# UCL-CCS/SCEMa

Measured on AMD Instinct MI355X. Metric: stress_evals_per_sec, higher is better.
Workload: dtype f64; 1 GPU; 576 x PE-10368 OPLS replicas per update(), 10+100 MD steps each (dt 2 fs, 300 K, lj/cut/coul/long 12/9 + PPPM 1e-4 + SHAKE + NVT), persistent per-QP state, replica equilibrated for 2000 steps before the timed region; force_field=opls, strain_set=balanced (load/unload: odd updates take the draw with the opposite sign), n_sims=576, atoms_per_replica=10368, sims_on_rank0=576, allgathers=0

## Files before the change

### include/scema_md.h

```cpp
#ifndef SCEMA_MD_H
#define SCEMA_MD_H

#include <stdint.h>

#ifdef __cplusplus
extern "C" {
#endif

#define SCEMA_MD_OK 0
#define SCEMA_MD_ERR_ARG 1
#define SCEMA_MD_ERR_NOSTATE 2
#define SCEMA_MD_ERR_DEVICE 3
#define SCEMA_MD_ERR_BOX 4
#define SCEMA_MD_ERR_IO 5
#define SCEMA_MD_ERR_OVERFLOW 6

#define SCEMA_MD_NPART 8
#define SCEMA_MD_QP_NONE ((int32_t)0xFFFFFFFF)

typedef struct scema_md_engine scema_md_engine;

typedef struct {
  double cut_lj;
  double cut_coul;
// ... 90 lines not shown
int scema_md_comm_init_rccl(scema_md_engine *e, const void *id, int32_t rank, int32_t world);
typedef int (*scema_md_host_allgather_fn)(void *ctx, const void *send, void *recv, int64_t bytes_per_rank);
typedef int (*scema_md_host_send_fn)(void *ctx, const void *buf, int64_t bytes, int32_t dst_rank);
typedef int (*scema_md_host_recv_fn)(void *ctx, void *buf, int64_t bytes, int32_t src_rank);
int scema_md_comm_init_host(scema_md_engine *e, int32_t rank, int32_t world, scema_md_host_allgather_fn allgather,
                            scema_md_host_send_fn send, scema_md_host_recv_fn recv, void *ctx);
void scema_md_comm_destroy(scema_md_engine *e);
int32_t scema_md_comm_world(const scema_md_engine *e);
int32_t scema_md_comm_rank(const scema_md_engine *e);
int scema_md_comm_stats(const scema_md_engine *e, int64_t *allgathers, int64_t *migrations);
int64_t scema_md_comm_handshakes(const scema_md_engine *e);
int32_t scema_md_state_owner(const scema_md_engine *e, int32_t qp_id, const char *matid, int32_t replica);

int scema_md_last_plan(const scema_md_engine *e, int32_t n_sims, int32_t *owner, int32_t *pos, int32_t *cap);
#define SCEMA_MD_RESULT_TRAILER 2
void *scema_md_local_stress_device_ptr(scema_md_engine *e);
int32_t scema_md_local_stress_count(const scema_md_engine *e);
int32_t scema_md_local_result_doubles(const scema_md_engine *e);
int scema_md_copy_local_stress(scema_md_engine *e, void *dst, int32_t dst_on_device);
int scema_md_scatter_gathered(scema_md_engine *e, const double *gathered, scema_mdsim *sims, int32_t n_sims);
int scema_md_settle_update(scema_md_engine *e, int32_t failed);
int64_t scema_md_unsettled_updates(const scema_md_engine *e);

typedef struct scema_plan_dir scema_plan_dir;
scema_plan_dir *scema_plan_dir_create(void);
void scema_plan_dir_destroy(scema_plan_dir *d);
int scema_plan_update(scema_plan_dir *d, const scema_mdsim *sims, int32_t n_sims, const double *cost, int32_t world,
                      int32_t *owner, int32_t *pos, int32_t *cap, int32_t *moves ,
                      int32_t *n_moves, int32_t commit);

int scema_md_has_state(const scema_md_engine *e, int32_t qp_id, const char *matid, int32_t replica);
int scema_md_get_state(scema_md_engine *e, int32_t qp_id, const char *matid, int32_t replica,
                       double box[9], double *x, double *v);
int scema_md_set_state(scema_md_engine *e, int32_t qp_id, const char *matid, int32_t replica,
                       const double box[9], const double *x, const double *v);
int scema_md_drop_state(scema_md_engine *e, int32_t qp_id, const char *matid, int32_t replica);
int scema_md_save_state_file(scema_md_engine *e, int32_t qp_id, const char *matid, int32_t replica, const char *path);
int scema_md_load_state_file(scema_md_engine *e, int32_t qp_id, const char *matid, int32_t replica, const char *path);
int scema_md_save_state_lammps(scema_md_engine *e, int32_t qp_id, const char *matid, int32_t replica, const char *path,
                               double timestep, int64_t ntimestep);

int scema_md_save_state_dump(scema_md_engine *e, int32_t qp_id, const char *matid, int32_t replica, const char *path,
                             int64_t ntimestep, int32_t precise);

typedef struct {
  double timestep_length;
  double temperature;
  int32_t nsteps_sample;
  double strain_ampl;
  double strain_rate;
} scema_md_eqparams;
int scema_md_init_material(scema_md_engine *e, const char *matid, int32_t replica, const scema_md_eqparams *p,
                           double length[3], double stress[6], double stiff[36]);

typedef struct {
  int32_t nsteps_equil;
  double timestep_length;
  double temperature;
  int64_t seed;
} scema_md_equilparams;
int scema_md_equilibrate(scema_md_engine *e, const char *matid, int32_t replica, const scema_md_equilparams *p, double length[3],
                         double *info);

int scema_md_debug_minimize(scema_md_engine *e, int32_t qp_id, const char *matid, int32_t replica, double etol, double ftol,
                            int32_t maxiter, int32_t maxeval, double *info);
int scema_md_debug_run_nh(scema_md_engine *e, int32_t qp_id, const char *matid, int32_t replica, int32_t nsteps, double dt,
                          double t_start, double t_stop, int32_t npt, double p_target, double p_period, double *lavg);
int scema_md_debug_compute(scema_md_engine *e, int32_t qp_id, const char *matid, int32_t replica, int32_t use_shake,
                           double *f, double *energies, double *virials, double *info );
int scema_md_debug_skin_bands(scema_md_engine *e, int32_t pos, uint64_t *out, int32_t cap);
int scema_md_debug_rows(scema_md_engine *e, int32_t pos, int32_t *cnt, int32_t *rows, int64_t rows_cap, int32_t *info);
int scema_md_debug_run(scema_md_engine *e, int32_t qp_id, const char *matid, int32_t replica, int32_t nsteps,
                       double dt, double temperature, int32_t nvt, int32_t use_shake, const double *rates,
                       double *press_avg);

int scema_md_reax_configure(scema_md_engine *e, const char *ffield_path, const char *const *elements, int32_t n_elements,
                            double qeq_tol, double skin);
int scema_md_reax_activate(scema_md_engine *e, int32_t on);
int scema_md_reax_set(scema_md_engine *e, int32_t exact_gradient, int32_t terms, int32_t qeq_maxiter);
int scema_md_reax_concurrency(scema_md_engine *e, int32_t halves, int32_t overlap);
int scema_md_batch_split(scema_md_engine *e, int32_t on);
int scema_md_get_concurrency(const scema_md_engine *e, int32_t *out);
int scema_md_pppm_tiling(scema_md_engine *e, int32_t mode, int32_t lds_bytes);
int scema_md_pppm_paths(const scema_md_engine *e, int32_t out[8]);
int scema_md_pppm_tile_shape(const int32_t grid[3], int32_t lds_bytes, int32_t which , int32_t out[4]);
int scema_md_pppm_plan_count(const scema_md_engine *e);
int scema_md_reax_debug_compute(scema_md_engine *e, int32_t qp_id, const char *matid, int32_t replica, double *f, double *eparts,
                                double *virial, double *q, double *info);
int scema_md_reax_stats(const scema_md_engine *e, double *out);

int scema_md_sw_configure(scema_md_engine *e, const char *matid, const char *sw_path, const char *const *elements, int32_t n_elements,
                          int32_t energy_unit, double skin);
int scema_md_sw_debug_compute(scema_md_engine *e, int32_t qp_id, const char *matid, int32_t replica, double *f, double *e2, double *e3,
                              double *virial, double *info);
int scema_md_sw_read_params(const char *sw_path, const char *const *elements, int32_t n_elements, int32_t energy_unit, int32_t *n_kept,
                            int32_t *type_map, double *values, char *errbuf, int32_t errcap);

int scema_md_tersoff_configure(scema_md_engine *e, const char *matid, const char *path, const char *const *elements, int32_t n_elements,
                               int32_t energy_unit, double skin);
int scema_md_tersoff_debug_compute(scema_md_engine *e, int32_t qp_id, const char *matid, int32_t replica, double *f, double *e_rep,
                                   double *e_att, double *virial, double *info);
int scema_md_tersoff_read_params(const char *path, const char *const *elements, int32_t n_elements, int32_t energy_unit, int32_t *n_kept,
                                 int32_t *type_map, double *values, char *errbuf, int32_t errcap);

int scema_md_tersoff_mod_configure(scema_md_engine *e, const char *matid, const char *path, const char *const *elements, int32_t n_elements,
                                   int32_t energy_unit, double skin);
int scema_md_tersoff_mod_debug_compute(scema_md_engine *e, int32_t qp_id, const char *matid, int32_t replica, double *f, double *e_rep,
                                       double *e_att, double *virial, double *info);
int scema_md_tersoff_zbl_configure(scema_md_engine *e, const char *matid, const char *path, const char *const *elements, int32_t n_elements,
                                   int32_t energy_unit, double skin);
int scema_md_tersoff_zbl_debug_compute(scema_md_engine *e, int32_t qp_id, const char *matid, int32_t replica, double *f, double *e_rep,
                                       double *e_att, double *virial, double *info);
int scema_md_tersoff_mod_read_params(const char *path, const char *const *elements, int32_t n_elements, int32_t energy_unit, int32_t *n_kept,
                                     int32_t *type_map, double *values, char *errbuf, int32_t errcap);
int scema_md_tersoff_zbl_read_params(const char *path, const char *const *elements, int32_t n_elements, int32_t energy_unit, int32_t *n_kept,
                                     int32_t *type_map, double *values, char *errbuf, int32_t errcap);

int scema_md_eam_configure(scema_md_engine *e, const char *matid, const char *path, const char *const *elements, int32_t n_elements,
                           int32_t energy_unit, double skin);
int scema_md_eam_debug_compute(scema_md_engine *e, int32_t qp_id, const char *matid, int32_t replica, double *f, double *e_pair,
                               double *e_embed, double *virial, double *info);
int scema_md_eam_read_setfl(const char *path, const char *const *elements, int32_t n_elements, int32_t energy_unit, int32_t *n_kept,
                            int32_t *type_map, double *head, double *masses, double *tables, int64_t tables_cap, char *errbuf, int32_t errcap);

int scema_md_vashishta_configure(scema_md_engine *e, const char *matid, const char *path, const char *const *elements, int32_t n_elements,
                                 int32_t energy_unit, double skin);
int scema_md_vashishta_debug_compute(scema_md_engine *e, int32_t qp_id, const char *matid, int32_t replica, double *f, double *e2, double *e3,
                                     double *virial, double *info);
int scema_md_vashishta_read_params(const char *path, const char *const *elements, int32_t n_elements, int32_t energy_unit, int32_t *n_kept,
                                   int32_t *type_map, double *values, char *errbuf, int32_t errcap);

int scema_md_adp_configure(scema_md_engine *e, const char *matid, const char *path, const char *const *elements, int32_t n_elements,
                           int32_t energy_unit, double skin);
int scema_md_adp_debug_compute(scema_md_engine *e, int32_t qp_id, const char *matid, int32_t replica, double *f, double *e_pair, double *e_manybody,
                               double *virial, double *info);
int scema_md_adp_read_setfl(const char *path, const char *const *elements, int32_t n_elements, int32_t energy_unit, int32_t *n_kept,
                            int32_t *type_map, double *head, double *masses, double *tables, int64_t tables_cap, char *errbuf, int32_t errcap);

int scema_md_edip_configure(scema_md_engine *e, const char *matid, const char *path, const char *const *elements, int32_t n_elements,
                            int32_t energy_unit, double skin);
int scema_md_edip_debug_compute(scema_md_engine *e, int32_t qp_id, const char *matid, int32_t replica, double *f, double *e2, double *e3,
                                double *virial, double *info);
int scema_md_edip_read_params(const char *path, const char *const *elements, int32_t n_elements, int32_t energy_unit, int32_t *n_kept,
                              int32_t *type_map, double *values, char *errbuf, int32_t errcap);

typedef struct {
  int64_t pair_launches;
  double pair_ms;
  double pair_alg_bytes;
  int64_t md_steps;
  int64_t neigh_builds;
  double unique_pairs_per_sim;
  int64_t evals;
  double list_skin_mean;
  int64_t pair_sims;
  int64_t box_flips;
  int64_t rx_sweep_launches;
  double rx_sweep_ms;
  double rx_sweep_entries;
  double rx_sweep_rows;
  int64_t rx_sweep_col_bytes;
  double pair_union_ms;
  double rx_sweep_union_ms;
  int64_t rx_sweep_symmetric;
  int64_t row_cell_builds;
} scema_md_profile;
// ... 14 lines not shown
```

### scema_amd/capi.py

```python
from __future__ import annotations

import ctypes as C
import os

import numpy as np

_HERE = os.path.dirname(os.path.abspath(__file__))
LIB_PATH = os.path.join(_HERE, os.environ.get("SCEMA_MD_LIB") or ("libscema_md_asan.so" if os.environ.get("SCEMA_SANITIZE") == "1" else "libscema_md.so"))

NPART = 8
PARTS = ["lj", "coul", "bond", "angle", "dihedral", "improper", "kspace", "shake"]
QP_NONE = -1

SYMBOLS = [
    "scema_md_default_params", "scema_md_create", "scema_md_destroy", "scema_md_last_error",
    "scema_md_register_replica", "scema_md_load_replica_file", "scema_md_write_replica_file",
    "scema_md_load_lammps_data", "scema_md_convert_lammps_data",
    "scema_md_probe_lammps_restart", "scema_md_read_lammps_restart_atoms", "scema_md_load_lammps_restart",
    "scema_md_convert_lammps_restart", "scema_md_write_lammps_restart",
    "scema_md_strain_batch", "scema_md_strain", "scema_md_local_stress_device_ptr",
    "scema_md_local_stress_count", "scema_md_local_result_doubles", "scema_md_copy_local_stress", "scema_md_scatter_gathered", "scema_md_settle_update", "scema_md_has_state", "scema_md_get_state",
    "scema_md_set_state", "scema_md_drop_state", "scema_md_save_state_file", "scema_md_load_state_file", "scema_md_save_state_lammps",
    "scema_md_init_material", "scema_md_debug_compute", "scema_md_debug_run", "scema_md_debug_skin_bands", "scema_md_debug_rows", "scema_md_get_profile", "scema_md_env_overrides",
    "scema_md_comm_unique_id", "scema_md_comm_init_rccl", "scema_md_comm_init_host", "scema_md_comm_destroy",
    "scema_md_comm_world", "scema_md_comm_rank", "scema_md_comm_stats", "scema_md_comm_handshakes", "scema_md_state_owner", "scema_md_last_plan",
    "scema_plan_dir_create", "scema_plan_dir_destroy", "scema_plan_update", "scema_md_kspace_setup",
    "scema_md_save_state_dump", "scema_md_replica_natoms", "scema_md_save_replica_file", "scema_md_equilibrate", "scema_md_debug_minimize", "scema_md_debug_run_nh",
    "scema_md_reax_configure", "scema_md_reax_activate", "scema_md_reax_set", "scema_md_reax_concurrency", "scema_md_batch_split", "scema_md_get_concurrency", "scema_md_pppm_plan_count", "scema_md_pppm_tiling", "scema_md_pppm_paths", "scema_md_pppm_tile_shape", "scema_md_unsettled_updates", "scema_md_reax_debug_compute", "scema_md_reax_stats", "scema_md_box_fma_tflops",
    "scema_md_sw_configure", "scema_md_sw_debug_compute", "scema_md_sw_read_params",
    "scema_md_tersoff_configure", "scema_md_tersoff_debug_compute", "scema_md_tersoff_read_params",
    "scema_md_eam_configure", "scema_md_eam_debug_compute", "scema_md_eam_read_setfl",
    "scema_md_tersoff_mod_configure", "scema_md_tersoff_mod_debug_compute", "scema_md_tersoff_mod_read_params",
    "scema_md_tersoff_zbl_configure", "scema_md_tersoff_zbl_debug_compute", "scema_md_tersoff_zbl_read_params",
    "scema_md_vashishta_configure", "scema_md_vashishta_debug_compute", "scema_md_vashishta_read_params",
    "scema_md_adp_configure", "scema_md_adp_debug_compute", "scema_md_adp_read_setfl",
    "scema_md_edip_configure", "scema_md_edip_debug_compute", "scema_md_edip_read_params",
]
COMM_ID_BYTES = 128
HOST_ALLGATHER_FN = C.CFUNCTYPE(C.c_int, C.c_void_p, C.c_void_p, C.c_void_p, C.c_int64)
HOST_SEND_FN = C.CFUNCTYPE(C.c_int, C.c_void_p, C.c_void_p, C.c_int64, C.c_int32)
HOST_RECV_FN = C.CFUNCTYPE(C.c_int, C.c_void_p, C.c_void_p, C.c_int64, C.c_int32)


class EquilParams(C.Structure):
    _fields_ = [("nsteps_equil", C.c_int32), ("timestep_length", C.c_double), ("temperature", C.c_double), ("seed", C.c_int64)]


class Params(C.Structure):
    _fields_ = [("cut_lj", C.c_double), ("cut_coul", C.c_double), ("skin", C.c_double), ("neigh_delay", C.c_int32),
                ("kspace_accuracy", C.c_double), ("shake_tol", C.c_double), ("shake_maxiter", C.c_int32),
                ("shake_mass", C.c_double), ("t_period", C.c_double), ("t_chain", C.c_int32), ("device", C.c_int32),
                ("max_batch", C.c_int32), ("profile", C.c_int32), ("kspace_style", C.c_int32)]


_P = C.c_void_p


class System(C.Structure):
    _fields_ = [("natoms", C.c_int32), ("ntypes", C.c_int32), ("type", _P), ("charge", _P), ("mass", _P),
                ("eps", _P), ("sigma", _P),
                ("nbonds", C.c_int32), ("nbondtypes", C.c_int32), ("bond_atoms", _P), ("bond_type", _P), ("bond_coeff", _P),
                ("nangles", C.c_int32), ("nangletypes", C.c_int32), ("angle_atoms", _P), ("angle_type", _P), ("angle_coeff", _P),
                ("ndihedrals", C.c_int32), ("ndihedraltypes", C.c_int32), ("dihedral_atoms", _P), ("dihedral_type", _P),
                ("dihedral_coeff", _P),
                ("nimpropers", C.c_int32), ("nimpropertypes", C.c_int32), ("improper_atoms", _P), ("improper_type", _P),
                ("improper_coeff", _P),
                ("special_lj", C.c_double * 3), ("special_coul", C.c_double * 3), ("box", C.c_double * 9), ("x", _P), ("v", _P)]


class MDSim(C.Structure):
    _fields_ = [("qp_id", C.c_int32), ("most_recent_qp_id", C.c_int32), ("replica", C.c_int32), ("material", C.c_int32),
                ("matid", C.c_char_p), ("time_id", C.c_char_p), ("output_folder", C.c_char_p),
                ("restart_folder", C.c_char_p), ("scripts_folder", C.c_char_p), ("log_file", C.c_char_p),
                ("force_field", C.c_char_p),
                ("strain", C.c_double * 6), ("stiffness", C.c_double * 36),
                ("timestep_length", C.c_double), ("temperature", C.c_double), ("strain_rate", C.c_double),
                ("nsteps_sample", C.c_int32), ("output_homog", C.c_int32), ("checkpoint", C.c_int32),
                ("stress", C.c_double * 6), ("stress_updated", C.c_int32)]


class EqParams(C.Structure):
    _fields_ = [("timestep_length", C.c_double), ("temperature", C.c_double), ("nsteps_sample", C.c_int32),
                ("strain_ampl", C.c_double), ("strain_rate", C.c_double)]


class Profile(C.Structure):
    _fields_ = [("pair_launches", C.c_int64), ("pair_ms", C.c_double), ("pair_alg_bytes", C.c_double),
                ("md_steps", C.c_int64), ("neigh_builds", C.c_int64), ("unique_pairs_per_sim", C.c_double),
                ("evals", C.c_int64), ("list_skin_mean", C.c_double), ("pair_sims", C.c_int64), ("box_flips", C.c_int64),
                ("rx_sweep_launches", C.c_int64), ("rx_sweep_ms", C.c_double), ("rx_sweep_entries", C.c_double), ("rx_sweep_rows", C.c_double), ("rx_sweep_col_bytes", C.c_int64),
                ("pair_union_ms", C.c_double), ("rx_sweep_union_ms", C.c_double), ("rx_sweep_symmetric", C.c_int64),
                ("row_cell_builds", C.c_int64)]


_lib = None


def lib():
    global _lib
    if _lib is None:
        if not os.path.exists(LIB_PATH):
            raise RuntimeError(f"{LIB_PATH} is missing: run `python -c 'import __graft_entry__ as g; g.build()'` "
                               "(make -C scema_amd/csrc); the engine has no CPU fallback")
        L = C.CDLL(LIB_PATH)
        L.scema_md_last_error.restype = C.c_char_p
        L.scema_md_last_error.argtypes = [_P]
        L.scema_md_local_stress_device_ptr.restype = C.c_void_p
        L.scema_md_local_stress_device_ptr.argtypes = [_P]
        L.scema_md_local_stress_count.argtypes = [_P]
        L.scema_md_destroy.argtypes = [_P]
        L.scema_md_destroy.restype = None
# ... 254 lines not shown
    def save_state_file(self, qp, matid, replica, path):
        self._chk(lib().scema_md_save_state_file(self.h, C.c_int32(qp), matid.encode(), C.c_int32(replica), path.encode()))

    def save_state_lammps(self, qp, matid, replica, path, timestep=2.0, ntimestep=0):
        self._chk(lib().scema_md_save_state_lammps(self.h, C.c_int32(qp), matid.encode(), C.c_int32(replica), path.encode(),
                                                   C.c_double(timestep), C.c_int64(ntimestep)))

    def save_state_dump(self, qp, matid, replica, path, ntimestep=0, precise=True):
        self._chk(lib().scema_md_save_state_dump(self.h, C.c_int32(qp), matid.encode(), C.c_int32(replica), path.encode(), C.c_int64(ntimestep),
                                                 C.c_int32(1 if precise else 0)))

    def load_state_file(self, qp, matid, replica, path):
        self._chk(lib().scema_md_load_state_file(self.h, C.c_int32(qp), matid.encode(), C.c_int32(replica), path.encode()))

    def debug_compute(self, matid, replica, qp=QP_NONE, use_shake=False):
        n = self._natoms[(matid, replica)]
        f = np.zeros((n, 3)); e = np.zeros(NPART); w = np.zeros((NPART, 6)); info = np.zeros(8)
        self._chk(lib().scema_md_debug_compute(self.h, C.c_int32(qp), matid.encode(), C.c_int32(replica),
                                               C.c_int32(1 if use_shake else 0), _p(f), _p(e), _p(w), _p(info)))
        return f, e, w, dict(g_ewald=info[0], nk=int(info[1]), npairs=info[2], tdof=info[3], t_current=info[4],
                             maxneigh_seen=int(info[5]), maxneigh=int(info[6]), nclus=int(info[7]))

    def debug_run(self, matid, replica, nsteps, dt, temperature, qp=QP_NONE, nvt=True, use_shake=True, rates=None, sample=False):
        r = None if rates is None else np.ascontiguousarray(rates, np.float64)
        pavg = np.zeros(6) if sample else None
        self._chk(lib().scema_md_debug_run(self.h, C.c_int32(qp), matid.encode(), C.c_int32(replica), C.c_int32(nsteps),
                                           C.c_double(dt), C.c_double(temperature), C.c_int32(1 if nvt else 0),
                                           C.c_int32(1 if use_shake else 0), _p(r), _p(pavg)))
        return pavg

    def debug_skin_bands(self, pos=0):
        out = np.zeros(64, np.uint64)
        self._chk(lib().scema_md_debug_skin_bands(self.h, C.c_int32(pos), out.ctypes.data_as(C.c_void_p), C.c_int32(out.size)))
        k = int(out[0])
        return dict(K=k, listed=[int(v) for v in out[1:1 + k]], walked=[int(v) for v in out[1 + k:1 + 2 * k]],
                    rows=int(out[1 + 2 * k]), rows_open=int(out[2 + 2 * k]), rows_all_open=int(out[3 + 2 * k]))

    def debug_rows(self, pos=0, rows=True):
        info = np.zeros(6, np.int32)
        f = lib().scema_md_debug_rows
        f.argtypes = [_P, C.c_int32, C.c_void_p, C.c_void_p, C.c_int64, C.c_void_p]
        self._chk(f(self.h, pos, None, None, 0, info.ctypes.data))
        out = dict(n=int(info[0]), cap=int(info[1]), cells=int(info[2]), ncell=[int(v) for v in info[3:6]])
        if rows:
            cnt = np.zeros(out["n"], np.int32)
            tab = np.zeros((out["n"], out["cap"]), np.int32)
            self._chk(f(self.h, pos, cnt.ctypes.data, tab.ctypes.data, tab.size, info.ctypes.data))
            out.update(cnt=cnt, rows=tab)
        return out

    def init_material(self, matid, replica, dt=2.0, temperature=300.0, nss=100, strain_ampl=0.005, strain_rate=1e-4):
        p = EqParams(dt, temperature, nss, strain_ampl, strain_rate)
        length, stress, stiff = np.zeros(3), np.zeros(6), np.zeros(36)
        self._chk(lib().scema_md_init_material(self.h, matid.encode(), C.c_int32(replica), C.byref(p), _p(length), _p(stress), _p(stiff)))
        return length, stress, stiff.reshape(6, 6)

    def reax_configure(self, ffield: str, elements=("H", "C", "N", "O"), qeq_tol: float = 1e-6, skin: float = -1.0):
        arr = (C.c_char_p * len(elements))(*[e.encode() for e in elements])
        self._chk(lib().scema_md_reax_configure(self.h, ffield.encode(), arr, C.c_int32(len(elements)), C.c_double(qeq_tol), C.c_double(skin)))

    def reax_activate(self, on: bool = True):
        self._chk(lib().scema_md_reax_activate(self.h, C.c_int32(1 if on else 0)))

    def reax_set(self, exact_gradient: int = -1, terms: int = -1, qeq_maxiter: int = -1):
        self._chk(lib().scema_md_reax_set(self.h, C.c_int32(exact_gradient), C.c_int32(terms), C.c_int32(qeq_maxiter)))

    def reax_concurrency(self, halves: int = -1, overlap: int = -1):
        self._chk(lib().scema_md_reax_concurrency(self.h, C.c_int32(halves), C.c_int32(overlap)))

    def unsettled_updates(self) -> int:
        lib().scema_md_unsettled_updates.restype = C.c_int64
        return int(lib().scema_md_unsettled_updates(self.h))

    def batch_split(self, on: int = -1):
        self._chk(lib().scema_md_batch_split(self.h, C.c_int32(on)))

    def pppm_plan_count(self) -> int:
        lib().scema_md_pppm_plan_count.restype = C.c_int
        return int(lib().scema_md_pppm_plan_count(self.h))

    def pppm_tiling(self, mode: int = -1, lds_bytes: int = -1):
        self._chk(lib().scema_md_pppm_tiling(self.h, C.c_int32(mode), C.c_int32(lds_bytes)))

    def pppm_paths(self) -> dict:
        out = (C.c_int32 * 8)()
        self._chk(lib().scema_md_pppm_paths(self.h, out))
        return dict(spread=int(out[0]), force=int(out[1]), spread_tiles=(int(out[2]), int(out[3])), force_tiles=(int(out[4]), int(out[5])),
                    lds_bytes=int(out[6]), mode=int(out[7]))

    def concurrency(self) -> dict:
        out = (C.c_int32 * 3)()
        self._chk(lib().scema_md_get_concurrency(self.h, out))
        return dict(split=int(out[0]), reax_halves=int(out[1]), reax_overlap=int(out[2]))

    def reax_compute(self, matid, replica, qp=QP_NONE):
        n = self._natoms[(matid, replica)]
        f = np.zeros((n, 3)); e = np.zeros(len(REAX_PARTS)); w = np.zeros(6); q = np.zeros(n); info = np.zeros(6)
        self._chk(lib().scema_md_reax_debug_compute(self.h, C.c_int32(qp), matid.encode(), C.c_int32(replica), _p(f), _p(e), _p(w), _p(q), _p(info)))
        return dict(f=f, e=dict(zip(REAX_PARTS, e)), w=w, q=q, maxneigh_seen=int(info[0]), maxnb=int(info[1]), maxbd=int(info[2]),
                    qeq_iters=int(info[3]), image_search=int(info[4]), maxbonds_seen=int(info[5]))

    def _row_configure(self, symbol, matid, path, elements, energy_unit, skin):
        arr = (C.c_char_p * len(elements))(*[e.encode() for e in elements])
        self._chk(getattr(lib(), symbol)(self.h, matid.encode(), path.encode(), arr, C.c_int32(len(elements)), C.c_int32(energy_unit), C.c_double(skin)))

    def _row_compute(self, symbol, matid, replica, qp, ea_key, eb_key, count_key):
        n = self.natoms(matid, replica)
        f = np.zeros((n, 3)); ea = C.c_double(0.0); eb = C.c_double(0.0); w = np.zeros(6); info = np.zeros(4)
        self._chk(getattr(lib(), symbol)(self.h, C.c_int32(qp), matid.encode(), C.c_int32(replica), _p(f), C.byref(ea), C.byref(eb), _p(w), _p(info)))
        return {"f": f, ea_key: ea.value, eb_key: eb.value, "w": w, "maxrow": int(info[0]), "rowcap": int(info[1]), "npairs": int(info[2]),
                count_key: int(info[3])}

    def sw_configure(self, matid: str, sw_path: str, elements=("Si",), energy_unit: int = 0, skin: float = -1.0):
        self._row_configure("scema_md_sw_configure", matid, sw_path, elements, energy_unit, skin)

    def sw_compute(self, matid, replica, qp=QP_NONE):
        return self._row_compute("scema_md_sw_debug_compute", matid, replica, qp, "e2", "e3", "ntriplets")

    def tersoff_configure(self, matid: str, path: str, elements=("Si",), energy_unit: int = 0, skin: float = -1.0):
        self._row_configure("scema_md_tersoff_configure", matid, path, elements, energy_unit, skin)

    def tersoff_compute(self, matid, replica, qp=QP_NONE):
        return self._row_compute("scema_md_tersoff_debug_compute", matid, replica, qp, "e_rep", "e_att", "nzeta")

    def tersoff_mod_configure(self, matid: str, path: str, elements=("Si",), energy_unit: int = 0, skin: float = -1.0):
        self._row_configure("scema_md_tersoff_mod_configure", matid, path, elements, energy_unit, skin)

    def tersoff_mod_compute(self, matid, replica, qp=QP_NONE):
        return self._row_compute("scema_md_tersoff_mod_debug_compute", matid, replica, qp, "e_rep", "e_att", "nzeta")

    def tersoff_zbl_configure(self, matid: str, path: str, elements=("Si",), energy_unit: int = 0, skin: float = -1.0):
        self._row_configure("scema_md_tersoff_zbl_configure", matid, path, elements, energy_unit, skin)

    def tersoff_zbl_compute(self, matid, replica, qp=QP_NONE):
        return self._row_compute("scema_md_tersoff_zbl_debug_compute", matid, replica, qp, "e_rep", "e_att", "nzeta")

    def vashishta_configure(self, matid: str, path: str, elements=("Si", "C"), energy_unit: int = 0, skin: float = -1.0):
        self._row_configure("scema_md_vashishta_configure", matid, path, elements, energy_unit, skin)

    def vashishta_compute(self, matid, replica, qp=QP_NONE):
        return self._row_compute("scema_md_vashishta_debug_compute", matid, replica, qp, "e2", "e3", "ntriplets")

    vashishta_debug_compute = vashishta_compute

    def eam_configure(self, matid: str, path: str, elements=("Cu",), energy_unit: int = 0, skin: float = -1.0):
        self._row_configure("scema_md_eam_configure", matid, path, elements, energy_unit, skin)

    def eam_compute(self, matid, replica, qp=QP_NONE):
        return self._row_compute("scema_md_eam_debug_compute", matid, replica, qp, "e_pair", "e_embed", "nabove")

    def edip_configure(self, matid: str, path: str, elements=("Si",), energy_unit: int = 0, skin: float = -1.0):
        self._row_configure("scema_md_edip_configure", matid, path, elements, energy_unit, skin)

    def edip_compute(self, matid, replica, qp=QP_NONE):
        return self._row_compute("scema_md_edip_debug_compute", matid, replica, qp, "e2", "e3", "ntriplets")

    edip_debug_compute = edip_compute

    def adp_configure(self, matid: str, path: str, elements=("Cu",), energy_unit: int = 0, skin: float = -1.0):
        self._row_configure("scema_md_adp_configure", matid, path, elements, energy_unit, skin)

    def adp_compute(self, matid, replica, qp=QP_NONE):
        return self._row_compute("scema_md_adp_debug_compute", matid, replica, qp, "e_pair", "e_manybody", "nabove")

    def minimize(self, matid, replica, qp, etol=1e-7, ftol=1e-11, maxiter=1000, maxeval=50000) -> dict:
        info = np.zeros(5)
# ... 225 lines not shown
```

### scema_amd/csrc/engine/engine.h

```cpp
#pragma once
#include <hip/hip_runtime.h>
#include <rccl/rccl.h>

#include <algorithm>
#include <cmath>
#include <cstdarg>
#include <cstdio>
#include <cstdlib>
#include <chrono>
#include <thread>
#include <cstring>
#include <ctime>
#include <array>
#include <atomic>
#include <functional>
#include <map>
#include <memory>
#include <sstream>
#include <fstream>
#include <string>
#include <vector>

#include "../../../include/scema_md.h"
#include "host/reax_ffield.h"
// ... 15 lines not shown
#include "md_adp.h"
#include "md_tersoff.h"
#include "md_vashishta.h"
#include "md_edip.h"
#include "md_rowcells.h"
#include "md_types.h"

namespace scema_eng {

struct DevBuf {
  void *p = nullptr;
  size_t bytes = 0;
  DevBuf() = default;
  DevBuf(const DevBuf &) = delete;
  DevBuf &operator=(const DevBuf &) = delete;
  ~DevBuf() { release(); }
  void release() {
    if (p) (void)hipFree(p);
    p = nullptr;
    bytes = 0;
  }
  hipError_t ensure(size_t n) {
    if (n <= bytes && p) return hipSuccess;
    release();
    if (n == 0) n = 8;
    hipError_t e = hipMalloc(&p, n);
    if (e == hipSuccess) bytes = n;
    return e;
  }
  template <class T>
  T *as() const { return reinterpret_cast<T *>(p); }
};

struct HostBox {
  double lo[3], h[6], hinv[6], vol;
};
inline void box_derive(const double *b, HostBox &o) {
  for (int d = 0; d < 3; d++) o.lo[d] = b[d];
  o.h[0] = b[3] - b[0]; o.h[1] = b[4] - b[1]; o.h[2] = b[5] - b[2];
  o.h[3] = b[8]; o.h[4] = b[7]; o.h[5] = b[6];
  o.hinv[0] = 1.0 / o.h[0]; o.hinv[1] = 1.0 / o.h[1]; o.hinv[2] = 1.0 / o.h[2];
  o.hinv[3] = -o.h[3] / (o.h[1] * o.h[2]);
  o.hinv[4] = (o.h[3] * o.h[5] - o.h[1] * o.h[4]) / (o.h[0] * o.h[1] * o.h[2]);
  o.hinv[5] = -o.h[5] / (o.h[0] * o.h[1]);
  o.vol = o.h[0] * o.h[1] * o.h[2];
}
inline void perp_widths(const HostBox &b, double w[3]) {
  w[0] = 1.0 / std::sqrt(b.hinv[0] * b.hinv[0] + b.hinv[5] * b.hinv[5] + b.hinv[4] * b.hinv[4]);
  w[1] = 1.0 / std::sqrt(b.hinv[1] * b.hinv[1] + b.hinv[3] * b.hinv[3]);
  w[2] = 1.0 / std::fabs(b.hinv[2]);
}

struct SysCopy {
  scema_md_system sys;
  std::vector<int32_t> type, ba, bt, aa, at, da, dt, ia, it;
  std::vector<double> q, mass, eps, sig, bc, ac, dc, ic;
  void take(const scema_md_system &s) {
    sys = s;
    const size_t n = (size_t)s.natoms, nt = (size_t)s.ntypes;
    type.assign(s.type, s.type + n); q.assign(s.charge, s.charge + n); mass.assign(s.mass, s.mass + nt);
    eps.assign(s.eps, s.eps + nt * nt); sig.assign(s.sigma, s.sigma + nt * nt);
    ba.assign(s.bond_atoms, s.bond_atoms + 2 * (size_t)s.nbonds); bt.assign(s.bond_type, s.bond_type + s.nbonds); bc.assign(s.bond_coeff, s.bond_coeff + 2 * (size_t)s.nbondtypes);
    aa.assign(s.angle_atoms, s.angle_atoms + 3 * (size_t)s.nangles); at.assign(s.angle_type, s.angle_type + s.nangles); ac.assign(s.angle_coeff, s.angle_coeff + 2 * (size_t)s.nangletypes);
    da.assign(s.dihedral_atoms, s.dihedral_atoms + 4 * (size_t)s.ndihedrals); dt.assign(s.dihedral_type, s.dihedral_type + s.ndihedrals); dc.assign(s.dihedral_coeff, s.dihedral_coeff + 4 * (size_t)s.ndihedraltypes);
    ia.assign(s.improper_atoms, s.improper_atoms + 4 * (size_t)s.nimpropers); it.assign(s.improper_type, s.improper_type + s.nimpropers); ic.assign(s.improper_coeff, s.improper_coeff + 2 * (size_t)s.nimpropertypes);
    sys.type = type.data(); sys.charge = q.data(); sys.mass = mass.data(); sys.eps = eps.data(); sys.sigma = sig.data();
    sys.bond_atoms = ba.data(); sys.bond_type = bt.data(); sys.bond_coeff = bc.data();
    sys.angle_atoms = aa.data(); sys.angle_type = at.data(); sys.angle_coeff = ac.data();
    sys.dihedral_atoms = da.data(); sys.dihedral_type = dt.data(); sys.dihedral_coeff = dc.data();
    sys.improper_atoms = ia.data(); sys.improper_type = it.data(); sys.improper_coeff = ic.data();
    sys.x = nullptr; sys.v = nullptr;
  }
};

inline unsigned long long next_object_id() { static std::atomic<unsigned long long> n{0}; return ++n; }
struct Topo {
  const unsigned long long id = next_object_id();
  int natoms = 0, ntypes = 0;
  SysCopy original;
  std::vector<int> type;
  std::vector<double> q, mass_atom, lj;
  int nbonds = 0, nbonds_noshake = 0, nangles = 0, ndihedrals = 0, nimpropers = 0, nspecial = 0, nclus = 0, ncons = 0, nfree = 0;
  double qsqsum = 0, qsum = 0, excl_cut = 0;
  double init_box[9];
  std::vector<double> init_x, init_v;
  DevBuf d_rtype;
  int rtype_stamp = -1;
  DevBuf d_type, d_q, d_mass, d_lj, d_bt_terms, d_bt_coef, d_ex_start, d_ex_list, d_clus_at, d_clus_n, d_clus_d, d_free_at, d_bt_desc, d_bt_atoms, d_bt_rank;
  int bt_ntile = 0, bt_maxloc = 1, bt_maxchunk = 1, bt_ncoef = 0, bt_cf_off[4] = {0, 0, 0, 0};
  double sp_w[6] = {0, 0, 0, 0, 0, 0};
  std::string matid;
  DevBuf d_eltype;
  long long eltype_stamp = 0;
};

struct State {
  const unsigned long long id = next_object_id();
  Topo *topo = nullptr;
  double box[9];
  DevBuf x, v;
  double skin_extra = 0.0;
  DevBuf qhist;
  bool qhist_valid = false;
};

struct RxSlot {
  int cap_pad = 0, cap_nb = 0, cap_bd = 0, cap_nbn = 0;
  size_t cap_col = 0;
  DevBuf nbn_cnt, nbn, nbnT, qpart, pm_len, pm_col, pm_raw, pm_val;
  DevBuf nb_cnt, nb_own0, nbT, hval, hcol, hlen, hown, hownlen, bd_cnt, bd, bd_rev, bd_bop, bd_c, bd_bo, bd_g, bd_cb, deltap, total_bo, cd_delta, hd, q, s, t, s_hist, t_hist, qwork, misc;
};

struct RowSlot {
  int cap_pad = 0;
  size_t cap_rows = 0;
  DevBuf cnt, rows, misc;
  DevBuf fp;
  DevBuf adp;
  int cap_cellpad = 0, cap_ncells = 0;
  DevBuf cstart, ccur, clist, cellof;
};

enum class RowKind { Opls, Reax, Sw, Tersoff, Eam, TersoffMod, TersoffZbl, Vashishta, Adp, Edip };

struct RowMaterial {
  RowKind kind = RowKind::Sw;
  std::vector<int> type_map;
  double cutmax = 0.0;
  double skin = 1.0;
  long long stamp = 0;
  DevBuf d_tab;
};

struct ListSig {
  bool valid = false;
  RowKind kind = RowKind::Opls;
  unsigned long long topo = 0;
  unsigned long long state = 0;
  int npad = 0;
  double rlist = 0.0;
  int nc[3] = {0, 0, 0}, capj = 0, maxneigh = 0;
  double cut_lj = 0.0, cut_coul = 0.0;
  long long stamp = 0;
  int mimg[3] = {0, 0, 0}, cap[2] = {0, 0};
  double corners_hold[24];
  int ago = 0, maxj_seen = 0;
  unsigned long long nentries = 0, nentries_ref = 0, nrowent = 0;
};
struct Slot {
  std::unique_ptr<RxSlot> rx;
  std::unique_ptr<RowSlot> row;
  ListSig sig;
  int cap_atoms = 0, cap_pad = 0, cap_neigh = 0, cap_cells = 0, cap_k = 0;
  size_t cap_jtab = 0;
  DevBuf virp, virb, fb, fs, slot_of, tile_nj, tile_jtab, tile_order, tile_wstart;
    DevBuf f, xq, stype, perm, slot_tmp, wrapn, xhold, cell_of, ckey, cell_count, cell_start, cell_fill, numneigh, dslot, neigh, sfac, kvec,
      xbak, vbak;
};

struct ActiveSim {
  State *st = nullptr;
  int user_index = -1;
  int nsteps = 0;
  double rates[6] = {0, 0, 0, 0, 0, 0};
  double dt = 0, temperature = 0;
  int nts = 0, nss = 0;
// ... 28 lines not shown

double event_union_ms(const std::vector<hipEvent_t> &ev, size_t n);
struct Profile {
  long long pair_launches = 0;
  double pair_ms = 0, pair_alg_bytes = 0;
  long long pair_sims = 0;
  double pair_union_ms = 0.0, rx_sweep_union_ms = 0.0;
  long long box_flips = 0;
  long long md_steps = 0, neigh_builds = 0, evals = 0;
  long long row_cell_builds = 0;
  double unique_pairs_sum = 0;
  long long unique_pairs_n = 0;
  double skin_sum = 0;
  long long rx_sweep_launches = 0;
  double rx_sweep_ms = 0, rx_sweep_entries = 0, rx_sweep_rows = 0;
  long long rx_sweep_col_bytes = 0, rx_sweep_symmetric = 0;
};

struct EwaldSetup {
  double g = 0.0;
  std::vector<int> kn;
  std::vector<int> krun;
  std::vector<int> kgrp;
  int kmaxd[3] = {0, 0, 0};
};

struct FlipEvent {
  int step;
  double tilt[3];
  int nflip[3];
};

struct RunSpec {
  int nvt = 1, use_shake = 1, deform = 0, sample = 0, ev_always = 0;
  int static_only = 0;
  int nh = 0, npt = 0, keep = 0, nh_total = 0, lavg_nav = 0;
  double t_start = 0, t_stop = 0, p_target = 1.0, p_period = 1000.0, box_margin = 0.0;
  std::vector<EwaldSetup> *ew_keep = nullptr;
  int minimize = 0, min_maxiter = 0, min_maxeval = 0;
  double min_etol = 0, min_ftol = 0;
  int keep_list = 0;
  int qeq_continue = 0;
};

struct EvalOpt {
  bool phase_a = true;
  int shake_a = 1, shake_b = 1;
};

}
using namespace scema_eng;

struct scema_md_engine {
  scema_md_params p;
  hipStream_t stream = nullptr;
  double skin_extra_fixed = 0.0;
  bool skin_adapt = false;
  hipStream_t stream2 = nullptr;
  hipStream_t stream3 = nullptr;
  hipEvent_t ev_up = nullptr;
  bool split_streams = true;
  hipEvent_t ev_fork = nullptr, ev_join = nullptr;
  bool rx_qeq_failed = false;
  long long rx_precond_fallbacks = 0;
  bool rx_precond = true;
  int rx_halves = 2, rx_overlap = 1;
  struct RxPart { hipStream_t main = nullptr, side = nullptr; hipEvent_t ev[4] = {nullptr, nullptr, nullptr, nullptr}; };
  std::vector<RxPart> rx_parts;
  std::vector<hipEvent_t> md_part_done;
  hipStream_t rx_side1 = nullptr;
  hipEvent_t rx_side1_ev[4] = {nullptr, nullptr, nullptr, nullptr};
  hipEvent_t row_fork = nullptr;
  std::map<std::string, std::unique_ptr<Topo>> topos;
  std::map<std::string, std::unique_ptr<State>> states;
  std::vector<std::unique_ptr<Slot>> slots;
  DevBuf d_sims, d_sc, d_local_stress, d_kpack, d_minptr, d_boxpair, d_pppm, d_copytab;
  std::vector<MdkCopy> h_copytab;
  DevBuf d_zerotab, d_rxstat;
  std::vector<MdkZero> h_zerotab;
  std::vector<long long> h_rxstat;
  std::vector<std::unique_ptr<DevBuf>> bak_x, bak_v;
  int pppm_tile_mode = 1, pppm_lds_bytes = 0;
  int pppm_paths[8] = {0, 0, 0, 0, 0, 0, 0, 1};
  std::map<std::array<int, 6>, hipfftHandle> pppm_plans;
  std::vector<int> h_kpack;
  int local_stress_count = 0;
  std::vector<SimDev> h_sims;
  std::vector<SimScalars> h_sc;
  std::vector<hipEvent_t> ev_pool;
  Profile prof;
  std::string err;
  double neigh_grow = 1.0;
  double jtab_grow = 1.0;
  int overflow_bits = 0;
  double overflow_need_j = 1.0, overflow_need_row = 1.0;
  long long unsettled_updates = 0;
  bool rx_ready = false, reax_active = false;
  int rx_stamp = 0;
  RxParams rx_host;
  std::vector<int> rx_type_map;
  DevBuf d_rxparams, d_rxviews;
  std::vector<RxView> h_rxviews;
  double rx_skin = 0.75, rx_qeq_tol = 1e-6;
  int rx_qeq_maxiter = 200, rx_terms = 31;
  bool rx_sym = true;
  long long rx_qeq_iters = 0, rx_qeq_solves = 0, rx_qeq_slow = 0;
  int rx_qeq_launch_cold = 48;
  int rx_qeq_launch = 32;
  bool rx_qeq_launch_pinned = false;
  std::map<std::string, std::unique_ptr<RowMaterial>> row_mats;
  long long row_stamp = 0;
  DevBuf d_rowviews;
  std::vector<RowView> h_rowviews;
  DevBuf d_eamviews;
  std::vector<EamView> h_eamviews;
  DevBuf d_adpviews;
  std::vector<AdpView> h_adpviews;
  DevBuf d_rowcells;
  std::vector<RowCells> h_rowcells;
  std::vector<unsigned char> h_rowcells_on;
  int rows_run_ns = 0;
  int row_cells_mode = 2;
  hipEvent_t row_part_done = nullptr;
  Comm comm;
  scema::OwnerDirectory dir;
  scema::SimPlan last_plan;
  PendingUpdate pending;
};

namespace scema_eng {

int fail(scema_md_engine *e, int code, const char *fmt, ...);

#define HIPCHK(call)                                                                                     \
  do {                                                                                                   \
    hipError_t _e = (call);                                                                              \
    if (_e != hipSuccess) return fail(e, SCEMA_MD_ERR_DEVICE, "%s failed: %s", #call, hipGetErrorString(_e)); \
  } while (0)
#define NCCLCHK(call)                                                                                         \
  do {                                                                                                    \
    ncclResult_t _r = (call);                                                                             \
    if (_r != ncclSuccess) return fail(e, SCEMA_MD_ERR_DEVICE, "%s failed: %s", #call, ncclGetErrorString(_r)); \
  } while (0)

std::string topo_key(const char *matid, int replica);
std::string state_key(int qp, const char *matid, int replica);

template <class T>
int upload(scema_md_engine *e, DevBuf &b, const std::vector<T> &v) {
  HIPCHK(b.ensure(v.size() * sizeof(T)));
  if (!v.empty()) HIPCHK(hipMemcpy(b.p, v.data(), v.size() * sizeof(T), hipMemcpyHostToDevice));
  return SCEMA_MD_OK;
}

int build_topo(scema_md_engine *e, const scema_md_system *s, Topo &t);
void ewald_setup(const scema_md_params &p, const Topo &t, const double *box, EwaldSetup &out, bool g_only = false);
void ewald_tables(EwaldSetup &out);
void pppm_setup_host(const scema_md_params &p, const Topo &t, const double *box, double &g, int pg[3]);
double cached_coul_poly(scema_md_engine *, double g, double rc, double *poly, int *npoly, double *uscale);
void tilt_closest(double tilt[3], double xprd_new, double yprd_new, double xy, double xz, double yz, double xprd, double yprd);
int tilt_flip(const double tilt[3], double xprd, double yprd, double flipped[3], int nflip[3]);
bool deform_trajectory(const double *box0, const double *rates, double dt, int nsteps, double *box_end, std::vector<FlipEvent> &events,
                       std::vector<HostBox> &extremes);
double wall_s();
double round_trip(const char *fmt, double v);
int settle_pending(scema_md_engine *e, bool failed);
// ... 115 lines not shown
```

### scema_amd/csrc/engine/engine_core.cpp

```cpp
#include <algorithm>
#include "engine.h"
#include "../md_env.h"

namespace scema_eng {

int fail(scema_md_engine *e, int code, const char *fmt, ...) {
  char buf[1024];
  va_list ap;
  va_start(ap, fmt);
  vsnprintf(buf, sizeof buf, fmt, ap);
  va_end(ap);
  if (e) e->err = buf;
  return code;
}

std::string topo_key(const char *matid, int replica) { return std::string(matid ? matid : "") + "_" + std::to_string(replica); }
std::string state_key(int qp, const char *matid, int replica) { return std::to_string(qp) + "." + topo_key(matid, replica); }

}

namespace scema_eng {
double event_union_ms(const std::vector<hipEvent_t> &ev, size_t n) {
  if (n == 0) return 0.0;
  std::vector<std::pair<float, float>> iv(n);
  for (size_t l = 0; l < n; l++) {
    float a = 0.f, b = 0.f;
    if (hipEventElapsedTime(&a, ev[0], ev[2 * l]) != hipSuccess || hipEventElapsedTime(&b, ev[0], ev[2 * l + 1]) != hipSuccess) return 0.0;
    iv[l] = {a, b};
  }
  std::sort(iv.begin(), iv.end());
  double total = 0.0;
  float lo = iv[0].first, hi = iv[0].second;
  for (size_t l = 1; l < n; l++) {
    if (iv[l].first > hi) { total += hi - lo; lo = iv[l].first; hi = iv[l].second; }
    else hi = std::max(hi, iv[l].second);
  }
  return total + (hi - lo);
}
}

namespace {
struct EnvSwitch { const char *name, *what; };
const EnvSwitch k_env[] = {
    {"SCEMA_MD_SPLIT", "0: never run a launch group of 9 simulations and more as part batches on streams of their own"},
    {"SCEMA_MD_PARTS", "2-4: this many part batches for every launch group that is split, if it has 2 replicas per part (default: by the size of the group, engine_run.cpp)"},
    {"SCEMA_MD_ONE_STREAM", "no side stream (bonded / k-space chain beside the pair kernel)"},
    {"SCEMA_MD_KEEP_LIST", "0: the sampling run of an evaluation rebuilds its neighbour rows at its start even where those of the straining run still hold"},
    {"SCEMA_MD_SKIN_BANDS", "0: the pair kernel walks every listed entry of a row on every step (default: the skin part of a row only as far as its cluster's and the replica's displacement bounds allow a pair inside the cutoff; results do not depend on it)"},
    {"SCEMA_MD_SKIN_EXTRA", "list skin = params.skin + this many Angstrom (results do not depend on it)"},
    {"SCEMA_MD_SKIN_ADAPT", "1: per-state adaptation of the extra skin from the rebuild interval (round-1 behaviour)"},
    {"SCEMA_MD_PPPM_SOLVE_WIDE", "1 / 0: the in-LDS PPPM solve with 1 024 threads and three LDS grids / 512 threads and two (default: by batch size)"},
    {"SCEMA_MD_PPPM_SOLVE_TWO", "0 / 1: the in-LDS PPPM solve of the 1 024-thread shape as one / two workgroups per replica, one per transform back (default: two for batches under 8 replicas)"},
    {"SCEMA_MD_PPPM_PADX", "0: the LDS grid of the PPPM spreading kernel without the five pad points per x row (an address addition per stencil point instead of a constant offset)"},
    {"SCEMA_MD_PPPM_FFT", "hipFFT for every PPPM grid (default: grids of up to 2 900 points are solved in LDS)"},
    {"SCEMA_MD_FUSED_TAIL", "0 / 1: force assembly + SHAKE + second kick as three kernels / as k_finish (default: by batch size)"},
    {"SCEMA_MD_BONDED_SIDE", "0: the bonded kernel of a small batch always on the main stream behind the pair kernel (default: behind the PPPM chain on the side stream on steps without a new influence function)"},
    {"SCEMA_MD_SMALL_BATCH_MAX", "largest batch that takes the cell grid with the most cells instead of the largest cells (default: launch groups of up to 31 replicas that run whole, i.e. not as part batches)"},
    {"SCEMA_MD_REBUILD_TOGETHER", "0 / 1: every replica rebuilds its neighbour rows on its own trigger / the replicas of a launch rebuild together as soon as one asks for it (default: together in launches of fewer than 128 replicas)"},
    {"SCEMA_MD_CELL_BUILD", "0: cell binning as k_bin + k_cell_scan + k_cell_fill instead of the one-launch k_cell_build"},
    {"SCEMA_MD_ROW_CELLS", "0 / 1: the neighbour rows of the row potentials never through cells (the N^2 build for every replica) / through cells wherever the geometry allows it, whatever the size (default: for no replica -- no measured size gains in the update time, DESIGN.md 7m; rows and results do not depend on it)"},
    {"SCEMA_MD_POLY_TOL", "fit target of the real-space Ewald polynomial (default 2e-13); parity tolerances assume the default"},
    {"SCEMA_REAX_DROP_DSBO2", "ReaxFF valence-angle gradient without the dSBO2 term, as USER-REAXC is believed to compute it"},
    {"SCEMA_MD_RX_ITEM_LDS", "0 (test hook): the ReaxFF angle and torsion items add forces and dE/dDelta to the work set with device-wide atomics instead of through a workgroup's LDS tables (replicas too large for the tables do)"},
    {"SCEMA_MD_RX_NEAR_FULL", "1 (test hook): the ReaxFF near rows hold every pair within the 5 A bond cutoff + skin instead of the pairs within reach of their type pair's bond order"},
    {"SCEMA_REAX_SKIN", "ReaxFF list skin in Angstrom"},
    {"SCEMA_REAX_HALVES", "number of part batches a ReaxFF batch runs as, each on its own stream (default 2; 0 or 1: one sequence of launches)"},
    {"SCEMA_REAX_OVERLAP", "0: the bond-order chain of the ReaxFF force stage on the same stream as the charge chain instead of next to it"},
    {"SCEMA_REAX_QEQ_PRECOND", "0: the conjugate gradients of the charge equilibration with the Jacobi preconditioner of fix qeq/reax instead of the bonded-pattern approximate inverse"},
    {"SCEMA_REAX_QEQ_SYM", "0: the matrix of the charge equilibration as full rows (every pair in both rows) instead of each pair once in its owner's row"},
    {"SCEMA_REAX_QEQ_ZLDS", "0: the matrix sweep of the charge equilibration gathers through the caches instead of from an LDS copy"},
    {"SCEMA_REAX_QEQ_LAUNCH", "conjugate-gradient iterations issued as launches per charge solve (default: adaptive)"},
    {"SCEMA_MD_NEIGH_GROW0", "start with undersized neighbour capacities: overflow -> restore -> regrow"},
    {"SCEMA_MD_NEIGH_EXACT", "1: every list build tests its candidates in FP64 at the exact list radius; 0: none does (default: the first build of a run)"},
    {"SCEMA_MD_TEST_FAIL_INCOMING", "rank on which the allocation of a state that migrates in fails (-1: on whichever rank receives one); the failure must reach every rank through the handshake"},
    {"SCEMA_MD_TEST_FAIL_MIGRATE", "<what>[:<rank>] -- an injected failure of the exchange of replica states: dbox / upload (before the handshake: every rank ends the call, nothing is posted), enqueue / group / hostcopy (after it: the exchange is completed, the error travels in the status word of the stress all-gather)"},
    {"SCEMA_MD_TEST_SELF_MOVE", "1 (RCCL, one rank): every simulation that continues from a state held here receives it through ncclSend / ncclRecv from this very rank"},
    {"SCEMA_MD_TEST_QEQ_PRECOND_FAILS", "1: a ReaxFF run whose charge solve uses the approximate-inverse preconditioner reports that it did not converge (the evaluation must come back from its one retry with the Jacobi preconditioner)"},
    {"SCEMA_MD_QCAP16", "capacity of k_neigh_build's group lists in sixteenths of the table: small values force the whole-table walk"},
    {"SCEMA_MD_RX_COL32", "32-bit column indices in the ReaxFF charge matrix whatever the replica size"},
    {"SCEMA_MD_RX_NB_ONCE", "0: the both-ends ReaxFF non-bonded kernel"},
    {"SCEMA_MD_RX_ITEMCAP", "capacity of the work-item lists of the ReaxFF angle and torsion kernels: small values force their in-place path"},
    {"SCEMA_MD_TIMING", "per-chunk wall times and the PAIR_TIMING / PAIR_COUNT counters on stderr"},
};
}

const char *scema_env(const char *name) {
  for (const EnvSwitch &s : k_env)
    if (strcmp(s.name, name) == 0) return getenv(name);
  fprintf(stderr, "[scema_md] environment switch %s is not declared in engine_core.cpp\n", name);
  abort();
}

extern "C" {

int scema_md_env_overrides(char *buf, int cap) {
  std::string out;
  int n = 0;
  for (const EnvSwitch &s : k_env)
    if (const char *v = getenv(s.name)) { out += (n ? "\n" : ""); out += s.name; out += "="; out += v; n++; }
  if (buf && cap > 0) { strncpy(buf, out.c_str(), (size_t)cap - 1); buf[cap - 1] = 0; }
  return n;
}

void scema_md_default_params(scema_md_params *p) {
  p->cut_lj = 12.0;
  p->cut_coul = 9.0;
  p->skin = 2.0;
  p->neigh_delay = 5;
  p->kspace_accuracy = 1.0e-4;
  p->shake_tol = 1.0e-3;
  p->shake_maxiter = 20;
  p->shake_mass = 1.0;
  p->t_period = 100.0;
  p->t_chain = 3;
  p->device = 0;
  p->max_batch = 0;
  p->profile = 0;
  p->kspace_style = 1;
}

int scema_md_create(const scema_md_params *p, scema_md_engine **out) {
  if (!out) return SCEMA_MD_ERR_ARG;
  *out = nullptr;
  scema_md_engine *e = new scema_md_engine();
  if (p) e->p = *p; else scema_md_default_params(&e->p);
  int ndev = 0;
  if (hipGetDeviceCount(&ndev) != hipSuccess || ndev <= 0) {
    delete e;
    return SCEMA_MD_ERR_DEVICE;
  }
  if (hipSetDevice(e->p.device) != hipSuccess || hipStreamCreateWithFlags(&e->stream, hipStreamNonBlocking) != hipSuccess) {
    delete e;
    return SCEMA_MD_ERR_DEVICE;
  }
  if (const char *sp = scema_env("SCEMA_MD_SPLIT")) e->split_streams = atoi(sp) != 0;
  if (hipStreamCreateWithFlags(&e->stream3, hipStreamNonBlocking) != hipSuccess || hipEventCreateWithFlags(&e->ev_up, hipEventDisableTiming) != hipSuccess)
// ... 105 lines not shown
```

### scema_amd/csrc/engine/engine_reax.cpp

```cpp
#include "engine.h"
#include "../md_env.h"

namespace scema_eng {


#define RXSET(dst, src) dst = (decltype(dst))(src)
static int ensure_rx_slot(scema_md_engine *e, RxSlot &r, int n, int npad, int maxnb, int maxbd, int maxnbn, bool col16) {
  if (npad > r.cap_pad) {
    HIPCHK(r.nb_cnt.ensure((size_t)npad * 4));
    HIPCHK(r.bd_cnt.ensure((size_t)npad * 4));
    HIPCHK(r.deltap.ensure((size_t)npad * 8));
    HIPCHK(r.total_bo.ensure((size_t)npad * 8));
    HIPCHK(r.cd_delta.ensure((size_t)npad * 8));
    HIPCHK(r.hd.ensure((size_t)npad * 8));
    HIPCHK(r.q.ensure((size_t)npad * 8));
    HIPCHK(r.s.ensure((size_t)npad * 8));
    HIPCHK(r.t.ensure((size_t)npad * 8));
    HIPCHK(r.s_hist.ensure(4 * (size_t)npad * 8));
    HIPCHK(r.t_hist.ensure(3 * (size_t)npad * 8));
    HIPCHK(r.qwork.ensure(10 * (size_t)npad * 8));
    HIPCHK(r.qpart.ensure((10 * (size_t)((npad + 255) / 256) + 2 * (size_t)(npad / RX_SWR + 1)) * 8));
    HIPCHK(r.pm_len.ensure((size_t)npad * 4));
    HIPCHK(r.pm_col.ensure((size_t)RX_PM_MAX * npad * 4));
    HIPCHK(r.pm_raw.ensure((size_t)RX_PM_MAX * npad * 8));
// ... 289 lines not shown
    if (on_pp) b += std::exp(t.p_bo5 * std::exp(t.p_bo6 * (lr - t.lr_pp)));
    return b;
  };
  if (!(P.bo_cut > 0.0) || bo(RX_BOND_CUT) >= P.bo_cut) return RX_BOND_CUT;
  double lo = 1e-3, hi = RX_BOND_CUT;
  if (bo(lo) < P.bo_cut) return lo;
  for (int it = 0; it < 200 && hi - lo > 1e-12; it++) {
    const double mid = 0.5 * (lo + hi);
    (bo(mid) >= P.bo_cut ? lo : hi) = mid;
  }
  return std::min((double)RX_BOND_CUT, hi * (1.0 + 1e-6) + 1e-6);
}
static void rx_near_radii(RxParams &P, double skin) {
  const bool full = scema_env("SCEMA_MD_RX_NEAR_FULL") && atoi(scema_env("SCEMA_MD_RX_NEAR_FULL")) != 0;
  for (int a = 0; a < RX_MAXT; a++)
    for (int b = 0; b < RX_MAXT; b++) {
      const bool used = a < P.nt && b < P.nt;
      const double reach = !used ? 0.0 : full ? (double)RX_BOND_CUT : std::max(rx_bond_reach(P, a, b), rx_bond_reach(P, b, a));
      if (used && b >= a && scema_env("SCEMA_MD_TIMING")) fprintf(stderr, "[scema_md] reax types %d-%d: bond order below bo_cut beyond %.4f A\n", a, b, reach);
      P.rbond[a * RX_MAXT + b] = reach;
      const double rn = std::max(reach, (double)RX_PM_RADIUS) + skin;
      P.rnear2[a * RX_MAXT + b] = used ? rn * rn : 0.0;
    }
}

int scema_md_reax_configure(scema_md_engine *e, const char *ffield_path, const char *const *elements, int32_t n_elements, double qeq_tol, double skin) {
  if (!e || !ffield_path || !elements || n_elements <= 0) return fail(e, SCEMA_MD_ERR_ARG, "bad arguments");
  HIPCHK(hipSetDevice(e->p.device));
  std::vector<std::string> el(elements, elements + n_elements);
  std::string err;
  RxParams P;
  std::vector<int> map;
  if (!scema::read_reax_ffield(ffield_path, el, P, map, err)) return fail(e, SCEMA_MD_ERR_IO, "%s", err.c_str());
  if (const char *x = scema_env("SCEMA_REAX_DROP_DSBO2")) P.lammps_dsbo2 = atoi(x) ? 1 : 0;
  e->rx_host = P;
  e->rx_type_map = map;
  if (qeq_tol > 0.0) e->rx_qeq_tol = qeq_tol;
  if (skin >= 0.0) e->rx_skin = skin;
  if (const char *x = scema_env("SCEMA_REAX_SKIN")) e->rx_skin = atof(x);
  if (const char *x = scema_env("SCEMA_REAX_QEQ_LAUNCH")) { e->rx_qeq_launch = e->rx_qeq_launch_cold = std::max(0, atoi(x)); e->rx_qeq_launch_pinned = true; }
  rx_near_radii(e->rx_host, e->rx_skin);
  HIPCHK(e->d_rxparams.ensure(sizeof(RxParams)));
  HIPCHK(hipMemcpyAsync(e->d_rxparams.p, &e->rx_host, sizeof(RxParams), hipMemcpyHostToDevice, e->stream));
  HIPCHK(hipStreamSynchronize(e->stream));
  e->rx_ready = true;
  e->rx_stamp += 1;
  e->reax_active = true;
  return SCEMA_MD_OK;
}
int scema_md_reax_activate(scema_md_engine *e, int32_t on) {
  if (!e) return SCEMA_MD_ERR_ARG;
  if (on && !e->rx_ready) return fail(e, SCEMA_MD_ERR_ARG, "no ReaxFF force field loaded");
  e->reax_active = on != 0;
  return SCEMA_MD_OK;
}
int scema_md_reax_concurrency(scema_md_engine *e, int32_t halves, int32_t overlap) {
  if (!e) return SCEMA_MD_ERR_ARG;
  if (halves >= 0) e->rx_halves = std::min(halves, 8);
  if (overlap >= 0) e->rx_overlap = overlap != 0;
  return SCEMA_MD_OK;
}
int scema_md_batch_split(scema_md_engine *e, int32_t on) {
  if (!e) return SCEMA_MD_ERR_ARG;
  if (on >= 0) e->split_streams = on != 0;
  return SCEMA_MD_OK;
}
int scema_md_get_concurrency(const scema_md_engine *e, int32_t *out) {
  if (!e || !out) return SCEMA_MD_ERR_ARG;
  out[0] = e->split_streams ? 1 : 0;
  out[1] = e->rx_halves;
  out[2] = e->rx_overlap ? 1 : 0;
  return SCEMA_MD_OK;
}
int scema_md_pppm_tiling(scema_md_engine *e, int32_t mode, int32_t lds_bytes) {
  if (!e) return SCEMA_MD_ERR_ARG;
  if (mode < -1 || mode > 1) return fail(e, SCEMA_MD_ERR_ARG, "scema_md_pppm_tiling: mode %d (1 tiled kernels, 0 the kernels without LDS, -1 keeps)", mode);
  const int least = 2 * 8, most = 160 * 1024;
  if (lds_bytes < -1 || (lds_bytes > 0 && (lds_bytes < least || lds_bytes > most)))
    return fail(e, SCEMA_MD_ERR_ARG, "scema_md_pppm_tiling: an LDS budget of %d bytes (%d .. %d, 0 the device default, -1 keeps)", lds_bytes, least, most);
  if (mode >= 0) e->pppm_tile_mode = mode;
  if (lds_bytes >= 0) e->pppm_lds_bytes = lds_bytes;
  return SCEMA_MD_OK;
}
int scema_md_pppm_paths(const scema_md_engine *e, int32_t out[8]) {
  if (!e || !out) return SCEMA_MD_ERR_ARG;
  for (int k = 0; k < 8; k++) out[k] = e->pppm_paths[k];
  return SCEMA_MD_OK;
}
int scema_md_pppm_tile_shape(const int32_t grid[3], int32_t lds_bytes, int32_t which, int32_t out[4]) {
  if (!grid || !out || grid[0] < 1 || grid[1] < 1 || grid[2] < 1 || lds_bytes < 0 || which < 0 || which > 1) return SCEMA_MD_ERR_ARG;
  const PppmTile t = pppm_tile_shape(grid[0], grid[1], grid[2], lds_bytes > 0 ? lds_bytes : (long long)mdk_pppm_lds_limit(), which);
  out[0] = t.by; out[1] = t.bz; out[2] = t.ty; out[3] = t.tz;
  return SCEMA_MD_OK;
}
int scema_md_pppm_plan_count(const scema_md_engine *e) { return e ? (int)e->pppm_plans.size() : -SCEMA_MD_ERR_ARG; }
int scema_md_reax_set(scema_md_engine *e, int32_t exact_gradient, int32_t terms, int32_t qeq_maxiter) {
  if (!e || !e->rx_ready) return fail(e, SCEMA_MD_ERR_ARG, "no ReaxFF force field loaded");
  HIPCHK(hipSetDevice(e->p.device));
  if (exact_gradient >= 0) {
    e->rx_host.lammps_dsbo2 = exact_gradient ? 0 : 1;
    HIPCHK(hipMemcpyAsync(e->d_rxparams.p, &e->rx_host, sizeof(RxParams), hipMemcpyHostToDevice, e->stream));
    HIPCHK(hipStreamSynchronize(e->stream));
  }
  if (terms >= 0) e->rx_terms = terms;
  if (qeq_maxiter > 0) e->rx_qeq_maxiter = qeq_maxiter;
  return SCEMA_MD_OK;
}
int scema_md_reax_debug_compute(scema_md_engine *e, int32_t qp_id, const char *matid, int32_t replica, double *f, double *eparts, double *virial,
                                double *q, double *info) {
  if (!e) return SCEMA_MD_ERR_ARG;
  if (!e->rx_ready) return fail(e, SCEMA_MD_ERR_ARG, "no ReaxFF force field loaded");
  HIPCHK(hipSetDevice(e->p.device));
  State *s = nullptr;
  std::unique_ptr<State> tmp;
  int rc = debug_state(e, qp_id, matid, replica, &s, tmp);
  if (rc) return rc;
  const bool saved = e->reax_active;
  e->reax_active = true;
  const long long it0 = e->rx_qeq_iters;
  RunSpec R;
  R.nvt = 0;
  R.static_only = 1;
  rc = eval_static(e, s, R);
  e->reax_active = saved;
  if (rc) return rc;
  const int n = s->topo->natoms;
  const SimScalars &sc = e->h_sc[0];
  const RxView &V = e->h_rxviews[0];
  if (f) HIPCHK(hipMemcpy(f, e->slots[0]->f.p, 3 * (size_t)n * 8, hipMemcpyDeviceToHost));
  if (eparts) HIPCHK(hipMemcpy(eparts, V.eparts, RX_NPART * 8, hipMemcpyDeviceToHost));
  if (q) HIPCHK(hipMemcpy(q, V.q, (size_t)n * 8, hipMemcpyDeviceToHost));
  if (virial)
    for (int k = 0; k < 6; k++) {
      virial[k] = 0.0;
      for (int p = 0; p < MD_NPART; p++) virial[k] += sc.vir[p * 6 + k];
    }
  if (info) {
    info[0] = sc.maxneigh_seen;
    info[1] = V.maxnb;
    info[2] = V.maxbd;
    info[3] = (double)(e->rx_qeq_iters - it0);
    info[4] = V.mimg[0] + V.mimg[1] + V.mimg[2];
    std::vector<int> bc(n);
    HIPCHK(hipMemcpy(bc.data(), V.bd_cnt, (size_t)n * 4, hipMemcpyDeviceToHost));
    int mb = 0;
    for (int v : bc) mb = std::max(mb, v);
    info[5] = mb;
  }
  return SCEMA_MD_OK;
}
int scema_md_reax_stats(const scema_md_engine *e, double *out) {
  if (!e || !out) return SCEMA_MD_ERR_ARG;
  out[0] = (double)e->rx_qeq_iters;
  out[1] = (double)e->rx_qeq_solves;
  out[2] = e->rx_skin;
  out[3] = e->rx_qeq_tol;
  out[4] = (double)e->rx_qeq_slow;
  out[5] = (double)e->rx_qeq_launch;
  out[6] = (double)e->rx_precond_fallbacks;
  return SCEMA_MD_OK;
}

}
```

### scema_amd/csrc/engine/engine_run.cpp

```cpp
#include "engine.h"
#include "../md_env.h"

namespace scema_eng {

static int padded_slots(int natoms, int ncells) { return (natoms + (MD_CLUSTER - 1) * ncells + 255) / 256 * 256; }

int ensure_slot(scema_md_engine *e, Slot &sl, int natoms, int maxneigh, int ncells, int nk, int capj) {
  const int npad = padded_slots(natoms, ncells);
  if (natoms > sl.cap_atoms || npad > sl.cap_pad) {
    HIPCHK(sl.f.ensure(3 * (size_t)natoms * 8));
    HIPCHK(sl.slot_of.ensure((size_t)natoms * 4));
    HIPCHK(sl.fs.ensure(3 * (size_t)npad * 8));
    HIPCHK(sl.fb.ensure(3 * (size_t)npad * 8));
    HIPCHK(sl.virb.ensure(((size_t)natoms / BT_OWNERS + 2) * 6 * 8));
    HIPCHK(sl.tile_order.ensure((size_t)npad * 4));
    HIPCHK(sl.wrapn.ensure(3 * (size_t)natoms * 4));
    HIPCHK(sl.xhold.ensure(3 * (size_t)natoms * 8));
    HIPCHK(sl.cell_of.ensure((size_t)natoms * 4));
    HIPCHK(sl.ckey.ensure((size_t)natoms * 4));
    HIPCHK(sl.slot_tmp.ensure((size_t)npad * 4));
    HIPCHK(sl.xbak.ensure(3 * (size_t)natoms * 8));
    HIPCHK(sl.vbak.ensure(3 * (size_t)natoms * 8));
    HIPCHK(sl.xq.ensure((size_t)npad * 32));
    HIPCHK(sl.stype.ensure((size_t)npad * 4));
    HIPCHK(sl.perm.ensure((size_t)npad * 4));
    HIPCHK(sl.numneigh.ensure((size_t)(npad / MD_CLUSTER) * MD_BAND_CNT * 2));
    HIPCHK(sl.dslot.ensure((size_t)npad * 4));
    sl.cap_atoms = natoms;
    sl.cap_pad = npad;
    sl.cap_neigh = 0;
  }
  if (maxneigh > sl.cap_neigh || sl.cap_neigh == 0) {
    HIPCHK(sl.neigh.ensure((size_t)maxneigh * (npad / MD_CLUSTER) * 4 + 8192));
    sl.cap_neigh = maxneigh;
  }
  if (ncells + 1 > sl.cap_cells) {
    HIPCHK(sl.cell_count.ensure((size_t)(ncells + 1) * 4));
    HIPCHK(sl.cell_start.ensure((size_t)(ncells + 1) * 4));
    HIPCHK(sl.cell_fill.ensure((size_t)(ncells + 1) * 4));
    HIPCHK(sl.tile_nj.ensure((size_t)(ncells + 1) * 4));
    HIPCHK(sl.tile_wstart.ensure((size_t)(ncells + 1) * 9 * 4));
    HIPCHK(sl.virp.ensure((size_t)(ncells + 1) * MD_TILE_WAVES * 6 * 8));
    sl.cap_cells = ncells + 1;
  }
  if ((size_t)ncells * capj > sl.cap_jtab || sl.cap_jtab == 0) {
    HIPCHK(sl.tile_jtab.ensure((size_t)ncells * capj * 4 + 1024));
    sl.cap_jtab = (size_t)ncells * capj;
  }
  if (nk > sl.cap_k || sl.cap_k == 0) {
    const int kc = std::max(nk, 64);
    HIPCHK(sl.sfac.ensure((size_t)kc * 2 * 8));
    HIPCHK(sl.kvec.ensure((size_t)kc * 4 * 8));
    sl.cap_k = kc;
  }
  return SCEMA_MD_OK;
}

namespace {

constexpr int MAXP = 4;

struct Policy {
  int kspace_threads = 1;
  int nparts = 1;
  int launch = 0;
  bool small_batch = false, nb_together = false, fuse_pack = false, keep_lists = true;
  bool pppm_in_lds = false, pppm_side = false, fused_tail = false, bonded_side = false, recip_side = false;
  bool recip_side_for(int na) const { return recip_side && na >= 16; }
};

Policy plan_launch(const scema_md_engine *e, int ns) {
  static const int parts_env = [] { const char *s = scema_env("SCEMA_MD_PARTS"); return s ? std::min(4, std::max(2, atoi(s))) : 0; }();
  static const int small_max = scema_env("SCEMA_MD_SMALL_BATCH_MAX") ? atoi(scema_env("SCEMA_MD_SMALL_BATCH_MAX")) : -1;
  static const int together_env = scema_env("SCEMA_MD_REBUILD_TOGETHER") ? atoi(scema_env("SCEMA_MD_REBUILD_TOGETHER")) : -1;
  Policy pol;
  pol.kspace_threads = ns >= 64 ? std::max(1, std::min(8, (int)std::thread::hardware_concurrency())) : 1;
  if (e->split_streams && e->stream3 != nullptr && ns >= 9) {
    pol.nparts = parts_env > 0 ? (ns >= 2 * parts_env ? parts_env : 2) : ns < 10 ? 3 : ns < 64 ? 4 : 2;
    if (e->stream2 == nullptr || e->rx_side1 == nullptr) pol.nparts = std::min(pol.nparts, 2);
    pol.nparts = std::max(1, std::min(pol.nparts, ns / 2));
  }
  pol.launch = (ns + pol.nparts - 1) / pol.nparts;
  pol.small_batch = small_max >= 0 ? ns <= small_max : (pol.nparts == 1 && ns <= 31);
  pol.nb_together = ns > 1 && (together_env < 0 ? pol.launch < 128 : together_env != 0);
  pol.fuse_pack = ns <= 32;
  pol.keep_lists = keep_list_switch();
  return pol;
}

struct Layout {
  int maxbt = 1, maxloc = 1, maxcoef = 0, maxrow = 64, maxcapj = 64, maxpoly = 1, maxatoms = 0, maxpad = 0, maxcells = 0, maxk = 0, mmax = 1,
      maxgrp = 0, maxclus = 0, maxunits = 0, maxsteps = 0;
  int maxgrid = 0, maxgridp = 0, maxdims = 0;
  bool padx_ok = true;
  PppmLaunch tl;
  bool tl_sp_fits = true, tl_fo_fits = true;
  bool any_validate = false;
};

void plan_sides(Policy &pol, const scema_md_engine *e, int ns, const RunSpec &spec, const Layout &L) {
  static const int fused_tail_env = scema_env("SCEMA_MD_FUSED_TAIL") ? atoi(scema_env("SCEMA_MD_FUSED_TAIL")) : -1;
  static const bool bonded_side_on = !(scema_env("SCEMA_MD_BONDED_SIDE") && atoi(scema_env("SCEMA_MD_BONDED_SIDE")) == 0);
  pol.pppm_in_lds = L.maxgrid > 0 && L.maxgrid <= mdk_pppm_solve_max() && (3 * (size_t)L.maxgrid + (size_t)L.maxdims) * 16 <= 150 * 1024 &&
                    !scema_env("SCEMA_MD_PPPM_FFT");
  pol.pppm_side = L.maxgrid > 0 && pol.nparts == 1 && e->stream2 != nullptr && ns < 256;
  pol.fused_tail = (fused_tail_env < 0 ? pol.launch <= 32 : fused_tail_env != 0) && !spec.nh && L.maxk == 0 && !spec.ev_always;
  pol.bonded_side = bonded_side_on && pol.pppm_side && pol.fused_tail && ns >= 8 && !(spec.deform || (spec.nh && spec.npt));
  pol.recip_side = pol.nparts == 1 && L.maxk > 0 && e->stream2 != nullptr;
}

using Clock = std::chrono::steady_clock;
double ms_between(Clock::time_point a, Clock::time_point b) { return std::chrono::duration<double, std::milli>(b - a).count(); }

struct OplsRun {
  scema_md_engine *e;
  std::vector<ActiveSim> &sims;
  const RunSpec &spec;
  const scema_md_params &P;
  const int ns;
  const double cutmax_all;
  const bool cle;
  const int ev;
  Policy pol;
  std::vector<int> order;
  std::vector<Part> parts;
  std::vector<EwaldSetup> ews;
  std::vector<std::vector<FlipEvent>> flips;
  std::vector<size_t> koff;
  Layout L;
  std::vector<std::pair<int, int>> pppm_runs;
  bool pppm_clean[MAXP] = {};
  const SimDev *D = nullptr;
  size_t ev_used = 0;
  std::vector<std::pair<int, int>> launch_sims;
  std::vector<std::unique_ptr<DevBuf>> flip_bufs;
  std::vector<std::unique_ptr<std::vector<int>>> flip_host;
  std::vector<std::unique_ptr<SimDev>> flip_desc;
  double t_layout = 0, t_kspace = 0, t_box = 0, t_grid = 0, t_rest = 0;

  OplsRun(scema_md_engine *e_, std::vector<ActiveSim> &sims_, const RunSpec &spec_)
      : e(e_), sims(sims_), spec(spec_), P(e_->p), ns((int)sims_.size()), cutmax_all(std::max(P.cut_lj, P.cut_coul)), cle(P.cut_coul <= P.cut_lj),
        ev((spec_.sample || spec_.ev_always || (spec_.nh && spec_.npt)) ? 1 : 0), pol(plan_launch(e_, (int)sims_.size())), flips(sims_.size()),
        koff(sims_.size(), 0) {
    L.tl.budget = e->pppm_lds_bytes > 0 ? e->pppm_lds_bytes : (int)mdk_pppm_lds_limit();
    L.tl.mode = e->pppm_tile_mode;
  }

  void kspace_setup();
  int make_parts();
  int lay_out_sim(int pos);
  int lay_out_kspace();
  int pppm_plan(const int pg[3], int batch, hipStream_t st, hipfftHandle &plan);
  int pppm_stage(hipStream_t st, int pos0, int na, bool new_box, int add = 1);
  int pppm_fork(hipStream_t st, int pos0, int na, bool new_box, bool with_bonded = false);
  hipError_t force_stage(hipStream_t st, const SimDev *Dh, int na, bool side, int bparts, int pairvir, bool pppm_ahead);
  int setup_step();
  int minimise();
  int launch_step(const Part &pt, int na, bool timed);
  int apply_flip(int pos, const FlipEvent &fe);
  int run_steps();
  int finish();
};

void OplsRun::kspace_setup() {
  std::vector<EwaldSetup> ews_i(ns);
  auto kspace_one = [&](int i) {
    const Topo &T = *sims[i].st->topo;
    const SimScalars &hsc = e->h_sc[i];
    EwaldSetup &ew = ews_i[i];
    const bool kept = spec.ew_keep && spec.keep;
    const bool pppm = P.kspace_style == 1 && T.qsqsum > 0.0 && !kept;
    if (kept && (int)spec.ew_keep->size() == ns) ew = (*spec.ew_keep)[i];
    else ewald_setup(P, T, hsc.box, ew, pppm);
    if (pppm) {
      int pgd[3];
      double gp = ew.g;
// ... 63 lines not shown

static bool choose_grid(const scema_md_engine *e, int natoms, const BoxRange &R, double rlist, bool small_batch, const ListSig *prev, SimDev &S,
                        int &capj, int &maxneigh, bool &keep) {
  keep = false;
  if (prev) {
    int mst[3], cj = 0, mn = 0;
    if (size_grid(e, natoms, R, rlist, prev->nc, mst, cj, mn) && cj <= prev->capj && mn <= prev->maxneigh &&
        padded_slots(natoms, prev->nc[0] * prev->nc[1] * prev->nc[2]) == prev->npad) {
      keep = true;
      capj = prev->capj; maxneigh = prev->maxneigh;
      for (int d = 0; d < 3; d++) { S.nc[d] = prev->nc[d]; S.mst[d] = mst[d]; }
      return true;
    }
  }
  bool fits = false;
  for (int pass = 0; pass < 2 && !fits; pass++) {
    int lo[3], hi[3];
    for (int d = 0; d < 3; d++) {
      lo[d] = std::max(2, std::min(64, (int)std::floor(R.w[d] / (rlist * 1.0001))));
      hi[d] = std::max(lo[d], std::min(64, (int)std::floor(R.w[d] / ((pass == 0 ? 0.5 : 0.25) * rlist * 1.0001))));
    }
    double best = -1.0e300;
    for (int n0 = lo[0]; n0 <= hi[0]; n0++)
      for (int n1 = lo[1]; n1 <= hi[1]; n1++)
        for (int n2 = lo[2]; n2 <= hi[2]; n2++) {
          const int nc[3] = {n0, n1, n2};
          int mst[3], cj, mn;
          if (!size_grid(e, natoms, R, rlist, nc, mst, cj, mn)) continue;
          const double score = small_batch ? (double)n0 * n1 * n2 : 1.0 / ((double)n0 * n1 * n2);
          if (score > best) {
            best = score;
            fits = true;
            capj = cj; maxneigh = mn;
            for (int d = 0; d < 3; d++) { S.nc[d] = nc[d]; S.mst[d] = mst[d]; }
          }
        }
  }
  for (int k = 5; k <= 8 && !fits; k++) {
    int nc[3], mst[3];
    for (int d = 0; d < 3; d++) nc[d] = std::max(1, std::min((int)std::floor(R.w[d] / (rlist / k * 1.0001)), 64));
    fits = size_grid(e, natoms, R, rlist, nc, mst, capj, maxneigh);
    for (int d = 0; d < 3; d++) { S.nc[d] = nc[d]; S.mst[d] = mst[d]; }
  }
  return fits;
}

int OplsRun::lay_out_sim(int pos) {
  const int i = order[pos];
  ActiveSim &A = sims[i];
  Topo &T = *A.st->topo;
  const SimScalars &hsc = e->h_sc[i];
  const auto tl0 = Clock::now();
  BoxRange R;
  if (!box_range(spec, A, hsc.box, R, flips[pos]))
    return fail(e, SCEMA_MD_ERR_BOX, "fix deform is changing yz too much with xy: the strain would tilt yz past half the box (a yz flip changes xz by xy, "
                "which LAMMPS refuses while xy is deformed too, as in.strain.lammps always does)");
  SimDev S;
  std::memset(&S, 0, sizeof S);
  if (!e->skin_adapt) A.st->skin_extra = e->skin_extra_fixed;
  for (int d = 0; d < 3; d++)
    if (R.w[d] < 2.0 * (cutmax_all + P.skin + A.st->skin_extra)) A.st->skin_extra = 0.0;
  const double skin_i = P.skin + A.st->skin_extra;
  const double rlist = cutmax_all + skin_i;
  for (int d = 0; d < 3; d++)
    if (R.w[d] < 2.0 * rlist) return fail(e, SCEMA_MD_ERR_BOX, "box width %.3f < 2*(cutoff+skin) = %.3f in dim %d", R.w[d], 2 * rlist, d);
  const auto tl1 = Clock::now();
  Slot &sl = *e->slots[i];
  const ListSig &g = sl.sig;
  const bool may_keep = spec.keep_list && pol.keep_lists && g.valid && g.kind == RowKind::Opls && g.topo == T.id && g.rlist == rlist && g.cut_lj == P.cut_lj &&
                        g.cut_coul == P.cut_coul && (spec.keep_list == 1 || g.state == A.st->id) && !hsc.force_rebuild && !hsc.overflow;
  int capj = 0, maxneigh = 0;
  bool keep = false;
  if (!choose_grid(e, T.natoms, R, rlist, pol.small_batch, may_keep ? &g : nullptr, S, capj, maxneigh, keep))
    return fail(e, SCEMA_MD_ERR_ARG, "the j table of a cell tile (%d entries) does not fit the LDS of the pair kernel (system too dense for the cutoff)", capj);
  S.keep_list = keep ? spec.keep_list : 0;
  L.any_validate = L.any_validate || S.keep_list != 0;
  S.ncells = S.nc[0] * S.nc[1] * S.nc[2];
  const auto tl2 = Clock::now();
  const EwaldSetup &ew = ews[pos];
  if (P.kspace_style == 1 && T.qsqsum > 0.0) {
    for (int d = 0; d < 3; d++) S.pg[d] = -ew.kmaxd[d];
    L.maxgrid = std::max(L.maxgrid, S.pg[0] * S.pg[1] * S.pg[2]);
    if (S.pg[0] < 5) L.padx_ok = false;
    L.maxgridp = std::max(L.maxgridp, (S.pg[0] + 5) * S.pg[1] * S.pg[2]);
    for (int which = 0; which < 2; which++) {
      const PppmTile t = pppm_tile_shape(S.pg[0], S.pg[1], S.pg[2], L.tl.budget, which);
      bool &fits = which ? L.tl_fo_fits : L.tl_sp_fits;
      if (t.ty == 0) { fits = false; continue; }
      int &my = which ? L.tl.fo_ty : L.tl.sp_ty, &mz = which ? L.tl.fo_tz : L.tl.sp_tz, &mt = which ? L.tl.fo_tiles : L.tl.sp_tiles;
      size_t &ml = which ? L.tl.fo_lds : L.tl.sp_lds;
      my = std::max(my, t.ty); mz = std::max(mz, t.tz); mt = std::max(mt, t.ty * t.tz);
      ml = std::max(ml, (size_t)pppm_tile_bytes(S.pg[0], S.pg[1], S.pg[2], t.by, t.bz, which));
    }
  }
  S.nk = (int)ew.kn.size() / 3;
  for (int d = 0; d < 3; d++) S.kmaxd[d] = std::max(ew.kmaxd[d], 0);
  S.g_ewald = ew.g;
  {
    const double perr = cached_coul_poly(e, ew.g, P.cut_coul, S.coul_poly, &S.coul_npoly, &S.coul_uscale);
    if (perr > 1e-12 && !scema_env("SCEMA_MD_POLY_TOL")) return fail(e, SCEMA_MD_ERR_ARG, "real-space Ewald polynomial fit error %.3e too large (g*rc = %.3f)", perr, ew.g * P.cut_coul);
    for (int m = 0; m < MD_MAXPOLY; m++) S.coul_poly_g[m] = S.coul_poly[m] * ew.g;
  }
  {
    const double m = 0.1 * P.skin;
    S.seg_a2 = (P.cut_coul + m) * (P.cut_coul + m);
    S.seg_b2 = (P.cut_lj + m) * (P.cut_lj + m);
    const double cmax = std::max(P.cut_coul, P.cut_lj);
    for (int b = 0; b < MD_SKIN_BANDS; b++) {
      const double w = m + b * (skin_i - m) / MD_SKIN_BANDS;
      S.band_e2[b] = (cmax + w) * (cmax + w);
      S.band_w[b] = skin_down(w);
    }
    S.dquant = (float)(skin_i / MD_DLEVELS);
    S.dquant_inv = (float)(MD_DLEVELS / skin_i);
    S.skin_bands = skin_bands_switch() ? 1 : 0;
  }
  S.natoms = T.natoms;
  S.npad = padded_slots(T.natoms, S.ncells);
  S.ntypes = T.ntypes;
  int rc = ensure_slot(e, sl, T.natoms, maxneigh, S.ncells, S.nk, capj);
  if (rc) return rc;
  S.maxneigh = maxneigh;
  S.capj = capj;
  {
    ListSig &gs = sl.sig;
    gs.valid = false;
    gs.kind = RowKind::Opls;
    gs.topo = T.id;
    for (int d = 0; d < 3; d++) gs.nc[d] = S.nc[d];
    gs.capj = capj; gs.maxneigh = maxneigh; gs.npad = S.npad;
    gs.rlist = rlist; gs.cut_lj = P.cut_lj; gs.cut_coul = P.cut_coul;
  }
  sim_common(S, P, spec, A, sl, e->d_sc.as<SimScalars>() + i);
  S.nbonds = T.nbonds; S.nbonds_noshake = T.nbonds_noshake; S.nangles = T.nangles; S.ndihedrals = T.ndihedrals;
  S.nimpropers = T.nimpropers; S.nspecial = T.nspecial; S.nclus = T.nclus;
  S.use_shake = (spec.use_shake && T.nclus > 0) ? 1 : 0;
  S.neigh_delay = P.neigh_delay;
  S.shake_maxiter = P.shake_maxiter;
  S.tdof = 3.0 * T.natoms - 3.0 - (S.use_shake ? T.ncons : 0);
  S.qsqsum = T.qsqsum; S.qsum = T.qsum;
  S.cut_lj2 = P.cut_lj * P.cut_lj; S.cut_coul2 = P.cut_coul * P.cut_coul; S.rlist2 = rlist * rlist;
  S.skin = skin_i;
  S.rlist_ref2 = (cutmax_all + P.skin) * (cutmax_all + P.skin);
  S.excl_cut2 = std::min(T.excl_cut * T.excl_cut, S.rlist2);
  S.shake_tol = P.shake_tol;
  S.lj = T.d_lj.as<double>();
  S.bt_terms = T.d_bt_terms.as<unsigned long long>(); S.bt_coef = T.d_bt_coef.as<double>(); S.bt_ncoef = T.bt_ncoef;
  for (int k = 0; k < 4; k++) S.bt_cf_off[k] = T.bt_cf_off[k];
  for (int k = 0; k < 6; k++) S.sp_w[k] = T.sp_w[k];
  S.ex_start = T.d_ex_start.as<int>(); S.ex_list = T.d_ex_list.as<int>();
  S.bt_desc = T.d_bt_desc.as<int>(); S.bt_atoms = T.d_bt_atoms.as<int>(); S.bt_rank = T.d_bt_rank.as<int>(); S.bt_ntile = T.bt_ntile;
  S.clus_at = T.d_clus_at.as<int>(); S.clus_n = T.d_clus_n.as<int>(); S.clus_d = T.d_clus_d.as<double>();
  S.free_at = T.d_free_at.as<int>(); S.nfree = T.nfree;
  S.xq = sl.xq.as<double4>(); S.stype = sl.stype.as<int>(); S.perm = sl.perm.as<int>(); S.slot_tmp = sl.slot_tmp.as<int>();
  S.cell_of = sl.cell_of.as<int>(); S.ckey = sl.ckey.as<int>(); S.cell_start = sl.cell_start.as<int>();
  S.cell_fill = sl.cell_fill.as<int>(); S.numneigh = sl.numneigh.as<int>(); S.neigh = sl.neigh.as<int>(); S.dslot = sl.dslot.as<float>();
  S.fs = sl.fs.as<double>(); S.fb = sl.fb.as<double>(); S.slot_of = sl.slot_of.as<int>(); S.tile_nj = sl.tile_nj.as<int>(); S.tile_jtab = sl.tile_jtab.as<int>(); S.tile_order = sl.tile_order.as<int>(); S.tile_wstart = sl.tile_wstart.as<int>(); S.virp = sl.virp.as<double>(); S.virb = sl.virb.as<double>();
  S.kvec = sl.kvec.as<double>();
  if (S.nk > 0) {
    std::vector<int> &kpack = e->h_kpack;
    koff[pos] = kpack.size();
    kpack.insert(kpack.end(), ew.kn.begin(), ew.kn.end());
    kpack.insert(kpack.end(), ew.krun.begin(), ew.krun.end());
    while (kpack.size() % 4) kpack.push_back(0);
    kpack.insert(kpack.end(), ew.kgrp.begin(), ew.kgrp.end());
    S.ngrp = (int)ew.kgrp.size() / 8;
    L.maxgrp = std::max(L.maxgrp, S.ngrp);
  }
  e->h_sims[pos] = S;
  t_box += ms_between(tl0, tl1); t_grid += ms_between(tl1, tl2); t_rest += ms_between(tl2, Clock::now());
  L.maxrow = std::max(L.maxrow, maxneigh); L.maxcapj = std::max(L.maxcapj, capj);
  L.maxbt = std::max(L.maxbt, T.bt_ntile); L.maxloc = std::max(L.maxloc, T.bt_maxloc); L.maxcoef = std::max(L.maxcoef, T.bt_ncoef);
  L.maxatoms = std::max(L.maxatoms, S.natoms); L.maxpad = std::max(L.maxpad, S.npad); L.maxcells = std::max(L.maxcells, S.ncells);
  L.maxk = std::max(L.maxk, S.nk);
  L.maxpoly = std::max(L.maxpoly, S.coul_npoly);
  for (int d = 0; d < 3; d++) L.mmax = std::max(L.mmax, S.kmaxd[d] + 1);
  L.maxclus = std::max(L.maxclus, S.use_shake ? S.nclus : 0);
  L.maxunits = std::max(L.maxunits, S.use_shake ? S.nclus + S.nfree : S.natoms);
  L.maxsteps = std::max(L.maxsteps, A.nsteps);
  return SCEMA_MD_OK;
}

int OplsRun::lay_out_kspace() {
  if ((size_t)64 * 3 * L.mmax * 16 + 4096 > 160 * 1024)
    return fail(e, SCEMA_MD_ERR_ARG, "k-space index range (|n| up to %d) too large for the LDS phase tables; raise cut_coul or loosen kspace_accuracy", L.mmax - 1);
  const std::vector<int> &kpack = e->h_kpack;
  HIPCHK(e->d_kpack.ensure(kpack.size() * sizeof(int) + 64));
  if (!kpack.empty()) HIPCHK(hipMemcpyAsync(e->d_kpack.p, kpack.data(), kpack.size() * sizeof(int), hipMemcpyHostToDevice, e->stream));
  for (int pos = 0; pos < ns; pos++) {
    SimDev &S = e->h_sims[pos];
    if (S.nk <= 0) continue;
    const int *base = e->d_kpack.as<int>() + koff[pos];
    S.kn = base;
    S.krun = base + 3 * (size_t)S.nk;
    S.kgrp = base + ((4 * (size_t)S.nk + 3) / 4) * 4;
  }
  if (!L.tl_sp_fits) L.tl.sp_tiles = 0;
  if (!L.tl_fo_fits) L.tl.fo_tiles = 0;
  if (L.maxgrid > 0) {
    const size_t mg = (size_t)L.maxgrid;
    const size_t gfs = mg + ((size_t)L.maxatoms + 1) / 2;
    HIPCHK(e->d_pppm.ensure((size_t)ns * (mg * 4 * sizeof(double2) + gfs * sizeof(double))));
    double *gbase = e->d_pppm.as<double>(), *ebase = gbase + (size_t)ns * mg * 2, *fbase = gbase + (size_t)ns * mg * 8;
    for (int pos = 0; pos < ns; pos++) {
      SimDev &S = e->h_sims[pos];
      S.pgrid = gbase + (size_t)pos * mg * 2;
      S.pfield = ebase + (size_t)pos * mg * 6;
      S.pgstride = (long long)L.maxgrid;
      S.pgf = fbase + (size_t)pos * gfs;
      L.maxdims = std::max(L.maxdims, S.pg[0] + S.pg[1] + S.pg[2]);
      const bool same = pos > 0 && pos != parts[part_of(parts, pos)].off && std::memcmp(S.pg, e->h_sims[pos - 1].pg, sizeof S.pg) == 0;
      if (same) pppm_runs.back().second += 1;
      else pppm_runs.push_back({pos, 1});
    }
  }
  return SCEMA_MD_OK;
}

int OplsRun::pppm_plan(const int pg[3], int batch, hipStream_t st, hipfftHandle &plan) {
  if ((long long)L.maxgrid > 0x7fffffffLL) return fail(e, SCEMA_MD_ERR_ARG, "PPPM grid of %d points is too large", L.maxgrid);
  const int sk = st == e->stream ? 0 : st == e->stream2 ? 1 : st == e->stream3 ? 2 : st == e->rx_side1 ? 3 : -1;
  if (sk < 0) return fail(e, SCEMA_MD_ERR_ARG, "PPPM transform on a stream the engine does not know");
  const std::array<int, 6> key = {pg[0], pg[1], pg[2], batch, sk, L.maxgrid};
  auto it = e->pppm_plans.find(key);
  if (it == e->pppm_plans.end()) {
    hipfftHandle h;
    int n[3] = {pg[2], pg[1], pg[0]};
    if (hipfftPlanMany(&h, 3, n, n, 1, L.maxgrid, n, 1, L.maxgrid, HIPFFT_Z2Z, batch) != HIPFFT_SUCCESS)
      return fail(e, SCEMA_MD_ERR_DEVICE, "hipfftPlanMany failed for a %d x %d x %d grid, batch %d", pg[0], pg[1], pg[2], batch);
    it = e->pppm_plans.emplace(key, h).first;
  }
  plan = it->second;
  return SCEMA_MD_OK;
}

int OplsRun::pppm_stage(hipStream_t st, int pos0, int na, bool new_box, int add) {
  if (L.maxgrid <= 0 || na <= 0) return SCEMA_MD_OK;
  const SimDev *Dp = D + pos0;
  bool &clean = pppm_clean[part_of(parts, pos0)];
  const int maxgridp = L.padx_ok ? L.maxgridp : 0;
  const int sp_path = mdk_pppm_spread_path(L.maxgrid, maxgridp, &L.tl), fo_path = mdk_pppm_force_path(L.maxgrid, &L.tl);
  {
    const int paths[8] = {sp_path, fo_path, sp_path == 1 ? L.tl.sp_ty : 1, sp_path == 1 ? L.tl.sp_tz : 1, fo_path == 1 ? L.tl.fo_ty : 1,
                          fo_path == 1 ? L.tl.fo_tz : 1, L.tl.budget, L.tl.mode};
    std::memcpy(e->pppm_paths, paths, sizeof paths);
  }
  if (sp_path == 1 || fo_path == 1) mdk_pppm_keys(st, Dp, na, L.maxatoms);
  mdk_pppm_spread(st, Dp, na, L.maxgrid, L.maxatoms, clean ? 1 : 0, maxgridp, &L.tl);
  clean = false;
  if (pol.pppm_in_lds) {
    if (new_box) mdk_pppm_gf(st, Dp, na, L.maxgrid);
    mdk_pppm_solve(st, Dp, na, L.maxgrid, L.maxdims);
    clean = true;
    mdk_pppm_force(st, Dp, na, L.maxgrid, L.maxatoms, add, 1, &L.tl);
    return SCEMA_MD_OK;
  }
  auto transform = [&](bool fields, int dir) -> int {
    for (const auto &run : pppm_runs) {
      if (run.first + run.second <= pos0 || run.first >= pos0 + na) continue;
      const SimDev &S0 = e->h_sims[run.first];
      if (S0.pg[0] == 0) continue;
      hipfftHandle plan;
      const int rc = pppm_plan(S0.pg, (fields ? 3 : 1) * run.second, st, plan);
      if (rc) return rc;
      double *g = fields ? S0.pfield : S0.pgrid;
      if (hipfftSetStream(plan, st) != HIPFFT_SUCCESS || hipfftExecZ2Z(plan, (hipfftDoubleComplex *)g, (hipfftDoubleComplex *)g, dir) != HIPFFT_SUCCESS)
        return fail(e, SCEMA_MD_ERR_DEVICE, "hipfftExecZ2Z failed");
    }
    return SCEMA_MD_OK;
  };
  int rc = transform(false, HIPFFT_FORWARD);
  if (rc) return rc;
  if (new_box) mdk_pppm_gf(st, Dp, na, L.maxgrid);
  mdk_pppm_poisson(st, Dp, na, L.maxgrid);
  if ((rc = transform(true, HIPFFT_BACKWARD))) return rc;
  mdk_pppm_force(st, Dp, na, L.maxgrid, L.maxatoms, add, 0, &L.tl);
  return SCEMA_MD_OK;
}

int OplsRun::pppm_fork(hipStream_t st, int pos0, int na, bool new_box, bool with_bonded) {
  if (!pol.pppm_side) return SCEMA_MD_OK;
  HIPCHK(hipEventRecord(e->ev_fork, st));
  HIPCHK(hipStreamWaitEvent(e->stream2, e->ev_fork, 0));
  const int rc = pppm_stage(e->stream2, pos0, na, new_box, 0);
  if (rc) return rc;
  if (with_bonded) mdk_bonded(e->stream2, D + pos0, na, L.maxbt, L.maxloc, L.maxcoef, 0);
  HIPCHK(hipEventRecord(e->ev_join, e->stream2));
  return SCEMA_MD_OK;
}

hipError_t OplsRun::force_stage(hipStream_t st, const SimDev *Dh, int na, bool side, int bparts, int pairvir, bool pppm_ahead) {
  hipError_t rc;
  if (side) {
    if ((rc = hipEventRecord(e->ev_fork, st)) != hipSuccess) return rc;
    if ((rc = hipStreamWaitEvent(e->stream2, e->ev_fork, 0)) != hipSuccess) return rc;
    mdk_ewald_recip(e->stream2, Dh, na, L.maxk, L.mmax, L.maxgrp);
    if ((rc = hipEventRecord(e->ev_join, e->stream2)) != hipSuccess) return rc;
  }
  mdk_bonded(st, Dh, na, L.maxbt, L.maxloc, L.maxcoef, bparts);
  if (side) {
    if ((rc = hipStreamWaitEvent(st, e->ev_join, 0)) != hipSuccess) return rc;
  } else {
    mdk_ewald_recip(st, Dh, na, L.maxk, L.mmax, L.maxgrp);
  }
  if (pppm_ahead) {
    if ((rc = hipStreamWaitEvent(st, e->ev_join, 0)) != hipSuccess) return rc;
  }
  mdk_ewald_force(st, Dh, na, L.maxatoms, pairvir, pppm_ahead ? 1 : 0);
  return hipSuccess;
}

int OplsRun::setup_step() {
  int rc = fork_parts(e, parts, e->ev_up);
  if (rc) return rc;
  for (const Part &pt : parts) {
    hipStream_t st = pt.st;
    const SimDev *Dh = D + pt.off;
    const int nh = pt.n;
    mdk_phase_init(st, Dh, nh);
    if (L.any_validate) mdk_keep_validate(st, Dh, nh, L.maxatoms);
    mdk_neighbor(st, Dh, nh, L.maxatoms, L.maxpad, L.maxcells, L.maxrow, L.maxcapj, true, pol.nb_together);
    if ((rc = pppm_fork(st, pt.off, nh, true))) return rc;
    mdk_pair(st, Dh, nh, L.maxcells, L.maxcapj, ev, spec.ev_always, L.maxpoly, cle);
    HIPCHK(force_stage(st, Dh, nh, pol.recip_side_for(nh), spec.ev_always, (ev && !spec.ev_always) ? 1 : 0, pol.pppm_side));
    if (!pol.pppm_side && (rc = pppm_stage(st, pt.off, nh, true))) return rc;
    if (!spec.static_only) mdk_shake(st, Dh, nh, L.maxclus, 0.5);
    mdk_final_integrate(st, Dh, nh, L.maxatoms, 0);
    if (spec.nh) mdk_setup_post_nh(st, Dh, nh);
    else mdk_setup_post(st, Dh, nh);
  }
  return SCEMA_MD_OK;
// ... 241 lines not shown
```

### scema_amd/csrc/engine/engine_topo.cpp

```cpp
#include "engine.h"

namespace scema_eng {

int build_topo(scema_md_engine *e, const scema_md_system *s, Topo &t) {
  const int n = s->natoms;
  if (n <= 0 || s->ntypes <= 0) return fail(e, SCEMA_MD_ERR_ARG, "natoms/ntypes out of range");
  if (n > MD_JMASK) return fail(e, SCEMA_MD_ERR_ARG, "too many atoms for the 27-bit neighbour index");
  t.natoms = n;
  const int nty = s->ntypes;
  std::vector<int> cls(nty, -1), rep;
  for (int u = 0; u < nty; u++) {
    for (size_t c = 0; c < rep.size() && cls[u] < 0; c++) {
      const int v = rep[c];
      bool same = true;
      for (int w = 0; w < nty && same; w++)
        same = s->eps[(size_t)u * nty + w] == s->eps[(size_t)v * nty + w] && s->sigma[(size_t)u * nty + w] == s->sigma[(size_t)v * nty + w] &&
               s->eps[(size_t)w * nty + u] == s->eps[(size_t)w * nty + v] && s->sigma[(size_t)w * nty + u] == s->sigma[(size_t)w * nty + v];
      if (same) cls[u] = (int)c;
    }
    if (cls[u] < 0) { cls[u] = (int)rep.size(); rep.push_back(u); }
  }
  const int ncls = (int)rep.size();
  if (ncls > MD_MAXTYPES) return fail(e, SCEMA_MD_ERR_ARG, "%d distinct Lennard-Jones types (of %d atom types): at most %d are supported", ncls, nty, MD_MAXTYPES);
  t.ntypes = ncls;
  t.type.resize(n);
  t.q.assign(s->charge, s->charge + n);
  t.mass_atom.resize(n);
  for (int i = 0; i < n; i++) {
    if (s->type[i] < 0 || s->type[i] >= nty) return fail(e, SCEMA_MD_ERR_ARG, "atom type out of range");
    t.type[i] = cls[s->type[i]];
    t.mass_atom[i] = s->mass[s->type[i]];
    t.qsqsum += t.q[i] * t.q[i];
    t.qsum += t.q[i];
  }
  const int nt2 = ncls * ncls;
  t.lj.resize(4 * nt2);
  for (int a = 0; a < ncls; a++)
    for (int b = 0; b < ncls; b++) {
      const size_t src = (size_t)rep[a] * nty + rep[b];
      const int k = a * ncls + b;
      const double s6 = std::pow(s->sigma[src], 6.0), s12 = s6 * s6;
      t.lj[k] = 48.0 * s->eps[src] * s12;
      t.lj[nt2 + k] = 24.0 * s->eps[src] * s6;
      t.lj[2 * nt2 + k] = 4.0 * s->eps[src] * s12;
      t.lj[3 * nt2 + k] = 4.0 * s->eps[src] * s6;
    }
  std::vector<std::vector<int>> adj(n);
  double max_r0 = 0.0;
  for (int b = 0; b < s->nbonds; b++) {
    const int a = s->bond_atoms[2 * b], c = s->bond_atoms[2 * b + 1];
    if (a < 0 || a >= n || c < 0 || c >= n || a == c) return fail(e, SCEMA_MD_ERR_ARG, "bad bond %d", b);
    adj[a].push_back(c);
    adj[c].push_back(a);
    max_r0 = std::max(max_r0, s->bond_coeff[2 * s->bond_type[b] + 1]);
  }
  std::vector<int> sp_at;
  std::vector<double> sp_cf;
  std::vector<std::vector<int>> excl(n);
  std::vector<int> level(n, 0), frontier, next, touched;
  int max_excl_level = 0;
  for (int i = 0; i < n; i++) {
    level[i] = -1;
    touched.assign(1, i);
    frontier.assign(1, i);
    for (int lvl = 1; lvl <= 3; lvl++) {
      next.clear();
      for (int a : frontier)
        for (int c : adj[a])
          if (level[c] == 0) {
            level[c] = lvl;
            next.push_back(c);
            touched.push_back(c);
          }
      frontier.swap(next);
    }
    for (int c : touched) {
      if (c > i) {
        const int lvl = level[c];
        const double wl = s->special_lj[lvl - 1], wc = s->special_coul[lvl - 1];
        if (!(wl == 1.0 && wc == 1.0)) {
          sp_at.push_back(i);
          sp_at.push_back(c);
          sp_cf.push_back(wl);
          sp_cf.push_back(wc);
          excl[i].push_back(c);
          excl[c].push_back(i);
          max_excl_level = std::max(max_excl_level, lvl);
        }
      }
    }
    for (int c : touched) level[c] = 0;
  }
  t.nspecial = (int)sp_cf.size() / 2;
  std::vector<int> ex_start(n + 1, 0), ex_list;
  for (int i = 0; i < n; i++) {
    std::sort(excl[i].begin(), excl[i].end());
    ex_start[i + 1] = ex_start[i] + (int)excl[i].size();
    ex_list.insert(ex_list.end(), excl[i].begin(), excl[i].end());
  }
  t.excl_cut = 1.5 * max_excl_level * max_r0;
  std::vector<char> shaken(s->nbonds, 0);
  std::vector<int> nsh(n, 0);
  if (e->p.shake_mass > 0.0)
    for (int b = 0; b < s->nbonds; b++) {
      const int a = s->bond_atoms[2 * b], c = s->bond_atoms[2 * b + 1];
      if (std::fabs(t.mass_atom[a] - e->p.shake_mass) <= 0.1 || std::fabs(t.mass_atom[c] - e->p.shake_mass) <= 0.1) {
        shaken[b] = 1;
        nsh[a]++;
        nsh[c]++;
      }
    }
  std::vector<int> cl_of(n, -1), clus_at, clus_n;
  std::vector<double> clus_d;
  for (int b = 0; b < s->nbonds; b++) {
    if (!shaken[b]) continue;
// ... 216 lines not shown
```

### scema_amd/csrc/md_pppm.h

```cpp
#pragma once
#include <hip/hip_runtime.h>
struct SimDev;
size_t mdk_pppm_lds_limit();
struct PppmLaunch {
  int budget = 0, mode = 1;
  int sp_ty = 0, sp_tz = 0, sp_tiles = 0, fo_ty = 0, fo_tz = 0, fo_tiles = 0;
  size_t sp_lds = 0, fo_lds = 0;
};
int mdk_pppm_spread_path(int maxgrid, int maxgridp, const PppmLaunch *tl);
int mdk_pppm_force_path(int maxgrid, const PppmLaunch *tl);
void mdk_pppm_keys(hipStream_t st, const SimDev *d, int ns, int maxatoms);
int mdk_pppm_spread(hipStream_t st, const SimDev *d, int ns, int maxgrid, int maxatoms, int zeroed, int maxgridp = 0, const PppmLaunch *tl = nullptr);
int mdk_pppm_solve_max();
void mdk_pppm_solve(hipStream_t st, const SimDev *d, int ns, int maxgrid, int maxdims);
void mdk_pppm_gf(hipStream_t st, const SimDev *d, int ns, int maxgrid);
void mdk_pppm_poisson(hipStream_t st, const SimDev *d, int ns, int maxgrid);
int mdk_pppm_force(hipStream_t st, const SimDev *d, int ns, int maxgrid, int maxatoms, int add, int real_fields = 0, const PppmLaunch *tl = nullptr);
```

### scema_amd/csrc/md_pppm.hip

```cpp
#include <hip/hip_runtime.h>

#include "md_device.h"
#include "md_env.h"
#include "md_pppm.h"
#include "md_pppm_tile.h"
#include "md_types.h"

#include <algorithm>
#include <cstdlib>

static inline dim3 grid2(int nx, int ns) { return dim3((unsigned)nx, (unsigned)ns, 1); }
static inline int cdiv(int a, int b) { return (a + b - 1) / b; }

#define PP_ORDER 5
#define PP_TPB 1024
#define PP_SOLVE_MAX 2900

static_assert(PP_ORDER == 5, "the blending polynomials below are those of order 5");
__device__ __forceinline__ int pppm_nearest(double u) { return (int)floor(u + 0.5); }
__device__ __forceinline__ void pppm_blend(double s, double (&w)[PP_ORDER]) {
  const double r = 1.0 - s;
  const double s2 = s * s, r2 = r * r;
  constexpr double q = 1.0 / 24.0;
  w[4] = q * (s2 * s2);
  w[0] = q * (r2 * r2);
  w[3] = fma(fma(fma(fma(-4.0 * q, s, 4.0 * q), s, 6.0 * q), s, 4.0 * q), s, q);
  w[2] = fma(fma(fma(fma(6.0 * q, s, -12.0 * q), s, -6.0 * q), s, 12.0 * q), s, 11.0 * q);
  w[1] = fma(fma(fma(fma(-4.0 * q, s, 12.0 * q), s, -6.0 * q), s, -12.0 * q), s, 11.0 * q);
}
__device__ __forceinline__ int pppm_weights(double u, double (&w)[PP_ORDER]) {
  const int i = pppm_nearest(u);
  pppm_blend(0.5 - ((double)i - u), w);
  return i;
}
__device__ __forceinline__ void pppm_weights_at(double u, int n, int km, double (&w)[PP_ORDER]) {
  const int i = (km == 0 && u >= 1.0) ? n : km;
  pppm_blend(0.5 - ((double)i - u), w);
}
__device__ __forceinline__ int pmod(int a, int n) { const int r = a % n; return r < 0 ? r + n : r; }
__device__ __forceinline__ void pppm_wrap(int i, int n, int (&g)[PP_ORDER]) {
#pragma unroll
  for (int k = 0; k < PP_ORDER; k++) {
    const int v = i + k - 2;
    g[k] = v < 0 ? v + n : (v >= n ? v - n : v);
  }
  if (n < 4)
#pragma unroll
    for (int k = 0; k < PP_ORDER; k++) g[k] = pmod(i + k - 2, n);
}
__device__ __forceinline__ void atom_lamda(const SimDev &S, const BoxD &b, int a, double &t0, double &t1, double &t2) {
  const double d0 = S.x[3 * a] - b.lo[0], d1 = S.x[3 * a + 1] - b.lo[1], d2 = S.x[3 * a + 2] - b.lo[2];
  const double l0 = b.hinv[0] * d0 + b.hinv[5] * d1 + b.hinv[4] * d2, l1 = b.hinv[1] * d1 + b.hinv[3] * d2, l2 = b.hinv[2] * d2;
  t0 = l0 - floor(l0); t1 = l1 - floor(l1); t2 = l2 - floor(l2);
}

__global__ __launch_bounds__(256) void k_pppm_zero(const SimDev *sims) {
  const SimDev &S = sims[blockIdx.y];
  const int NG = S.pg[0] * S.pg[1] * S.pg[2], idx = blockIdx.x * 256 + threadIdx.x;
  if (idx < NG) ((double2 *)S.pgrid)[idx] = make_double2(0.0, 0.0);
}

extern __shared__ double s_grid[];
template <bool LDS, int TPB_, bool PADX = false>
__global__ __launch_bounds__(TPB_) void k_pppm_spread(const SimDev *sims, int split) {
  const SimDev &S = sims[blockIdx.y];
  const int nx = S.pg[0], ny = S.pg[1], nz = S.pg[2];
  if (nx == 0) return;
  const int NG = nx * ny * nz, T = (int)blockDim.x;
  const int nxp = PADX ? nx + 5 : nx, NGP = nxp * ny * nz;
  const int chunk = (S.natoms + split - 1) / split, a0 = (int)blockIdx.x * chunk, a1 = min(S.natoms, a0 + chunk);
  if (a0 >= a1) return;
  BoxD b;
  box_derive(S.sc->box, b);
  box_uniform(b);
  double2 *rho = (double2 *)S.pgrid;
  if (LDS) {
    for (int k = threadIdx.x; k < NGP; k += T) s_grid[k] = 0.0;
    __syncthreads();
  }
  const double delvolinv = (double)NG / b.vol;
  const int rows = (a1 - a0 + 63) >> 6, lane = threadIdx.x & 63;
  for (int r = 2 * ((int)threadIdx.x >> 6); r < rows; r += 2 * (T >> 6)) {
    const int aA = a0 + lane * rows + r, aB = aA + 1;
    const bool vA = aA < a1, vB = r + 1 < rows && aB < a1;
    if (!vA) continue;
    double wxA[PP_ORDER], wyA[PP_ORDER], wzA[PP_ORDER], wxB[PP_ORDER] = {0, 0, 0, 0, 0}, wyB[PP_ORDER] = {0, 0, 0, 0, 0}, wzB[PP_ORDER] = {0, 0, 0, 0, 0};
    int gxA[PP_ORDER], gyA[PP_ORDER], gzA[PP_ORDER], gxB[PP_ORDER] = {0, 0, 0, 0, 0}, gyB[PP_ORDER] = {0, 0, 0, 0, 0}, gzB[PP_ORDER] = {0, 0, 0, 0, 0};
    double l0, l1, l2;
    atom_lamda(S, b, aA, l0, l1, l2);
    const int ixA = pppm_weights(l0 * nx, wxA), iyA = pppm_weights(l1 * ny, wyA), izA = pppm_weights(l2 * nz, wzA);
    pppm_wrap(ixA, nx, gxA); pppm_wrap(iyA, ny, gyA); pppm_wrap(izA, nz, gzA);
    const double zA = delvolinv * S.q[aA];
    double zB = 0.0;
    int ixB = -1000, iyB = 0, izB = 0;
    if (vB) {
      atom_lamda(S, b, aB, l0, l1, l2);
      ixB = pppm_weights(l0 * nx, wxB); iyB = pppm_weights(l1 * ny, wyB); izB = pppm_weights(l2 * nz, wzB);
      pppm_wrap(ixB, nx, gxB); pppm_wrap(iyB, ny, gyB); pppm_wrap(izB, nz, gzB);
      zB = delvolinv * S.q[aB];
    }
    const bool merged = vB && ixA == ixB && iyA == iyB && izA == izB;
#pragma unroll
    for (int k = 0; k < PP_ORDER; k++) { wxA[k] *= zA; if (vB) wxB[k] *= zB; }
    if (zA != 0.0 || (merged && zB != 0.0)) {
#pragma unroll
      for (int c = 0; c < PP_ORDER; c++) {
#pragma unroll
        for (int bb = 0; bb < PP_ORDER; bb++) {
          const double zyA = wzA[c] * wyA[bb], zyB = merged ? wzB[c] * wyB[bb] : 0.0;
          const int row = (gzA[c] * ny + gyA[bb]) * nxp;
          double *prow = s_grid + row + ixA;
#pragma unroll
          for (int k = 0; k < PP_ORDER; k++) {
            const double val = fma(zyB, wxB[k], zyA * wxA[k]);
            if (LDS && PADX) (void)__hip_atomic_fetch_add(prow + k, val, __ATOMIC_RELAXED, __HIP_MEMORY_SCOPE_WORKGROUP);
            else if (LDS) (void)__hip_atomic_fetch_add(&s_grid[row + gxA[k]], val, __ATOMIC_RELAXED, __HIP_MEMORY_SCOPE_WORKGROUP);
            else atomicAdd(&rho[row + gxA[k]].x, val);
          }
        }
      }
    }
    if (vB && !merged && zB != 0.0) {
#pragma unroll
      for (int c = 0; c < PP_ORDER; c++) {
#pragma unroll
        for (int bb = 0; bb < PP_ORDER; bb++) {
          const double zyB = wzB[c] * wyB[bb];
          const int row = (gzB[c] * ny + gyB[bb]) * nxp;
          double *prow = s_grid + row + ixB;
#pragma unroll
          for (int k = 0; k < PP_ORDER; k++) {
            if (LDS && PADX) (void)__hip_atomic_fetch_add(prow + k, zyB * wxB[k], __ATOMIC_RELAXED, __HIP_MEMORY_SCOPE_WORKGROUP);
            else if (LDS) (void)__hip_atomic_fetch_add(&s_grid[row + gxB[k]], zyB * wxB[k], __ATOMIC_RELAXED, __HIP_MEMORY_SCOPE_WORKGROUP);
            else atomicAdd(&rho[row + gxB[k]].x, zyB * wxB[k]);
          }
        }
      }
    }
  }
  if (LDS) {
    __syncthreads();
    if (PADX) {
      const int nrow = ny * nz;
      for (int k = threadIdx.x; k < 5 * nrow; k += T) {
        const int row = k / 5, pc = k - 5 * row;
        const int src = pc < 2 ? pc : nx + pc, dst = (pc < 2 ? nx - 2 + pc : pc - 2) + 2;
        s_grid[row * nxp + dst] += s_grid[row * nxp + src];
      }
      __syncthreads();
      for (int k = threadIdx.x; k < NG; k += T) {
        const int row = k / nx, x = k - row * nx;
        const double v = s_grid[row * nxp + x + 2];
        if (split == 1) rho[k] = make_double2(v, 0.0);
        else if (v != 0.0) atomicAdd(&rho[k].x, v);
      }
    } else if (split == 1) {
      for (int k = threadIdx.x; k < NG; k += T) rho[k] = make_double2(s_grid[k], 0.0);
    } else {
      for (int k = threadIdx.x; k < NG; k += T) {
        const double v = s_grid[k];
        if (v != 0.0) atomicAdd(&rho[k].x, v);
      }
    }
  }
}

__device__ __forceinline__ double sinc_pow10(double x) {
  if (x == 0.0) return 1.0;
  const double s = sin(x) / x, s2 = s * s, s4 = s2 * s2;
  return s4 * s4 * s2;
}
__global__ __launch_bounds__(256) void k_pppm_gf(const SimDev *sims) {
  const SimDev &S = sims[blockIdx.y];
  const int nx = S.pg[0], ny = S.pg[1], nz = S.pg[2];
  if (nx == 0) return;
  const int NG = nx * ny * nz, idx = blockIdx.x * 256 + threadIdx.x;
  if (idx >= NG) return;
  const int m1 = idx % nx, m2 = (idx / nx) % ny, m3 = idx / (nx * ny);
  const int p1 = m1 - nx * (2 * m1 / nx), p2 = m2 - ny * (2 * m2 / ny), p3 = m3 - nz * (2 * m3 / nz);
  if (p1 == 0 && p2 == 0 && p3 == 0) { S.pgf[idx] = 0.0; return; }
  BoxD b;
  box_derive(S.sc->box, b);
  const double twopi = 2.0 * MD_PI;
  const double kx = twopi * (b.hinv[0] * p1), ky = twopi * (b.hinv[5] * p1 + b.hinv[1] * p2), kz = twopi * (b.hinv[4] * p1 + b.hinv[3] * p2 + b.hinv[2] * p3);
  const double sqk = kx * kx + ky * ky + kz * kz, g2inv4 = 0.25 / (S.g_ewald * S.g_ewald);
  double wxs[5], wys[5], wzs[5];
#pragma unroll
  for (int a = 0; a < 5; a++) {
    wxs[a] = sinc_pow10(MD_PI * (double)(p1 + nx * (a - 2)) / nx);
    wys[a] = sinc_pow10(MD_PI * (double)(p2 + ny * (a - 2)) / ny);
    wzs[a] = sinc_pow10(MD_PI * (double)(p3 + nz * (a - 2)) / nz);
  }
  double num = 0.0, den = 0.0;
  for (int a3 = 0; a3 < 5; a3++)
    for (int a2 = 0; a2 < 5; a2++) {
      const int q2 = p2 + ny * (a2 - 2), q3 = p3 + nz * (a3 - 2);
      const double w23 = wys[a2] * wzs[a3];
#pragma unroll
      for (int a1 = 0; a1 < 5; a1++) {
        const int q1 = p1 + nx * (a1 - 2);
        const double qx = twopi * (b.hinv[0] * q1), qy = twopi * (b.hinv[5] * q1 + b.hinv[1] * q2), qz = twopi * (b.hinv[4] * q1 + b.hinv[3] * q2 + b.hinv[2] * q3);
        const double dot2 = qx * qx + qy * qy + qz * qz;
        const double w2 = wxs[a1] * w23;
        den += w2;
        num += (kx * qx + ky * qy + kz * qz) / dot2 * exp(-dot2 * g2inv4) * w2;
      }
    }
  S.pgf[idx] = 4.0 * MD_PI / sqk * num / (den * den);
}

__device__ __forceinline__ double2 pppm_mode(const SimDev &S, const BoxD &b, int idx, int nx, int ny, int nz, double2 r, double (&kv)[3], double (&v)[6], double &e) {
  const int NG = nx * ny * nz;
  const int m1 = idx % nx, m2 = (idx / nx) % ny, m3 = idx / (nx * ny);
  const int p1 = m1 - nx * (2 * m1 / nx), p2 = m2 - ny * (2 * m2 / ny), p3 = m3 - nz * (2 * m3 / nz);
  const double twopi = 2.0 * MD_PI;
  const double kx = twopi * (b.hinv[0] * p1), ky = twopi * (b.hinv[5] * p1 + b.hinv[1] * p2), kz = twopi * (b.hinv[4] * p1 + b.hinv[3] * p2 + b.hinv[2] * p3);
  kv[0] = kx; kv[1] = ky; kv[2] = kz;
  const double gf = S.pgf[idx], scaleinv = 1.0 / (double)NG;
  const double ar = r.x * scaleinv, ai = r.y * scaleinv;
  if (gf != 0.0) {
    const double sqk = kx * kx + ky * ky + kz * kz;
    const double eg = 0.5 * b.vol * MD_QQRD2E * gf * (ar * ar + ai * ai);
    const double vterm = -2.0 * (1.0 / sqk + 0.25 / (S.g_ewald * S.g_ewald));
    e += eg;
    v[0] += eg * (1.0 + vterm * kx * kx); v[1] += eg * (1.0 + vterm * ky * ky); v[2] += eg * (1.0 + vterm * kz * kz);
    v[3] += eg * vterm * kx * ky; v[4] += eg * vterm * kx * kz; v[5] += eg * vterm * ky * kz;
  }
  if (idx == 0)
    e -= MD_QQRD2E * (S.g_ewald * S.qsqsum / sqrt(MD_PI) + 0.5 * MD_PI * S.qsum * S.qsum / (S.g_ewald * S.g_ewald * b.vol));
  return make_double2(gf * ar, gf * ai);
}

__global__ __launch_bounds__(256) void k_pppm_poisson(const SimDev *sims) {
  const SimDev &S = sims[blockIdx.y];
  const int nx = S.pg[0], ny = S.pg[1], nz = S.pg[2];
  if (nx == 0) return;
  __shared__ double s_red[8 * 4];
  const int NG = nx * ny * nz, idx = blockIdx.x * 256 + threadIdx.x;
  if ((int)(blockIdx.x * 256) >= NG) return;
  double v[6] = {0, 0, 0, 0, 0, 0}, e[1] = {0};
  BoxD b;
  box_derive(S.sc->box, b);
  if (idx < NG) {
    double kv[3];
    const double2 p = pppm_mode(S, b, idx, nx, ny, nz, ((const double2 *)S.pgrid)[idx], kv, v, e[0]);
    const size_t gs = (size_t)S.pgstride;
    double2 *field = (double2 *)S.pfield;
// ... 114 lines not shown
    }
    __syncthreads();
  }
  if (BGLOBAL)
    for (int k = threadIdx.x; k < NG; k += PP_SOLVE_TPB) rho[k] = make_double2(0.0, 0.0);
  if (c_lo == 0) {
    block_atomic_add_n<6, PP_SOLVE_TPB / 64>(v, S.sc->vir + P_KSPACE * 6, s_red);
    block_atomic_add_n<1, PP_SOLVE_TPB / 64>(e, S.sc->eng + P_KSPACE, s_red);
  }
#ifdef PAIR_TIMING
  PP_CLK();
  if (threadIdx.x == 0 && blockIdx.x == 0 && blockIdx.y == 0 && ntq == 8) {
    for (int k = 1; k < 8; k++) atomicAdd(&S.sc->dbg2[k - 1], tq[k] - tq[k - 1]);
    atomicAdd(&S.sc->dbg2[7], 1ull);
  }
#endif
#undef PP_CLK
}

template <bool LDS, bool REALF = false>
__global__ __launch_bounds__(256) void k_pppm_force(const SimDev *sims, int split, int add) {
  const SimDev &S = sims[blockIdx.y];
  const int nx = S.pg[0], ny = S.pg[1], nz = S.pg[2];
  if (nx == 0) return;
  const int NG = nx * ny * nz;
  int chunk = (S.natoms + split - 1) / split;
  chunk = (chunk + 255) & ~255;
  const int a0 = (int)blockIdx.x * chunk, a1 = min(S.natoms, a0 + chunk);
  if (a0 >= a1) return;
  const size_t gs = (size_t)S.pgstride;
  const double2 *ex = (const double2 *)S.pfield, *ey = ex + gs, *ez = ey + gs;
  if (LDS) {
    if (REALF) {
      const double *fr = (const double *)S.pfield;
      for (int k = threadIdx.x; k < NG; k += 256) { s_grid[k] = fr[k]; s_grid[NG + k] = fr[gs + k]; s_grid[2 * NG + k] = fr[2 * gs + k]; }
    } else {
      for (int k = threadIdx.x; k < NG; k += 256) { s_grid[k] = ex[k].x; s_grid[NG + k] = ey[k].x; s_grid[2 * NG + k] = ez[k].x; }
    }
    __syncthreads();
  }
  BoxD b;
  box_derive(S.sc->box, b);
  box_uniform(b);
  for (int a = a0 + (int)threadIdx.x; a < a1; a += 256) {
    const double qa = S.q[a];
    if (qa == 0.0) {
      if (!add) { S.f[3 * a] = 0.0; S.f[3 * a + 1] = 0.0; S.f[3 * a + 2] = 0.0; }
      continue;
    }
    double l0, l1, l2;
    atom_lamda(S, b, a, l0, l1, l2);
    double wx[PP_ORDER], wy[PP_ORDER], wz[PP_ORDER];
    int gx[PP_ORDER], gy[PP_ORDER], gz[PP_ORDER];
    pppm_wrap(pppm_weights(l0 * nx, wx), nx, gx);
    pppm_wrap(pppm_weights(l1 * ny, wy), ny, gy);
    pppm_wrap(pppm_weights(l2 * nz, wz), nz, gz);
    double fx = 0.0, fy = 0.0, fz = 0.0;
#pragma unroll
    for (int c = 0; c < PP_ORDER; c++) {
#pragma unroll
      for (int bb = 0; bb < PP_ORDER; bb++) {
        const double zy = wz[c] * wy[bb];
        const int row = (gz[c] * ny + gy[bb]) * nx;
        double rx = 0.0, ry = 0.0, rz = 0.0;
#pragma unroll
        for (int k = 0; k < PP_ORDER; k++) {
          const int g = row + gx[k];
          if (LDS) { rx = fma(wx[k], s_grid[g], rx); ry = fma(wx[k], s_grid[NG + g], ry); rz = fma(wx[k], s_grid[2 * NG + g], rz); }
          else if (REALF) { const double *fr = (const double *)S.pfield; rx = fma(wx[k], fr[g], rx); ry = fma(wx[k], fr[gs + g], ry); rz = fma(wx[k], fr[2 * gs + g], rz); }
          else { rx = fma(wx[k], ex[g].x, rx); ry = fma(wx[k], ey[g].x, ry); rz = fma(wx[k], ez[g].x, rz); }
        }
        fx = fma(zy, rx, fx); fy = fma(zy, ry, fy); fz = fma(zy, rz, fz);
      }
    }
    const double qf = MD_QQRD2E * qa;
    if (add) { S.f[3 * a] += qf * fx; S.f[3 * a + 1] += qf * fy; S.f[3 * a + 2] += qf * fz; }
    else { S.f[3 * a] = qf * fx; S.f[3 * a + 1] = qf * fy; S.f[3 * a + 2] = qf * fz; }
  }
}


#define PP_KEY_Y(key) ((key) & 0xffff)
#define PP_KEY_Z(key) (((key) >> 16) & 0x7fff)
__device__ __forceinline__ int MD_G *pppm_keys_of(const SimDev &S) { return (int MD_G *)(S.pgf + S.pgstride); }
__global__ __launch_bounds__(256) void k_pppm_keys(const SimDev *sims) {
  const SimDev &S = sims[blockIdx.y];
  if (S.pg[0] == 0) return;
  const int ny = S.pg[1], nz = S.pg[2], a = blockIdx.x * 256 + threadIdx.x;
  if (a >= S.natoms) return;
  BoxD b;
  box_derive(S.sc->box, b);
  box_uniform(b);
  double l0, l1, l2;
  atom_lamda(S, b, a, l0, l1, l2);
  const int iy = pmod(pppm_nearest(l1 * ny), ny), iz = pmod(pppm_nearest(l2 * nz), nz);
  pppm_keys_of(S)[a] = iy | (iz << 16) | (S.q[a] == 0.0 ? (int)0x80000000 : 0);
}
struct PppmBrick { int y0, z0, byc, bzc, hy, hz; };
__device__ __forceinline__ bool pppm_brick(int nx, int ny, int nz, int budget, int which, PppmBrick &B) {
  const PppmTile t = pppm_tile_shape(nx, ny, nz, budget, which);
  const int tile = (int)blockIdx.x;
  if (tile >= t.ty * t.tz) return false;
  const int tzi = tile / t.ty, tyi = tile - tzi * t.ty;
  B.y0 = tyi * t.by; B.z0 = tzi * t.bz;
  B.byc = min(t.by, ny - B.y0); B.bzc = min(t.bz, nz - B.z0);
  B.hy = t.by < ny ? 4 : 0; B.hz = t.bz < nz ? 4 : 0;
  return true;
}
__device__ __forceinline__ int pppm_rel(int a, int b, int d, int n) {
  const int v = a - b + d;
  return v < 0 ? v + n : (v >= n ? v - n : v);
}

template <int TPB_>
__global__ __launch_bounds__(TPB_) void k_pppm_spread_tiled(const SimDev *sims, int budget) {
  const SimDev &S = sims[blockIdx.y];
  const int nx = S.pg[0], ny = S.pg[1], nz = S.pg[2];
  if (nx == 0) return;
  PppmBrick B;
  if (!pppm_brick(nx, ny, nz, budget, 0, B)) return;
  const int y0 = B.y0, z0 = B.z0, byc = B.byc, bzc = B.bzc;
  const int NG = nx * ny * nz, NB = nx * byc * bzc, T = TPB_;
  for (int k = threadIdx.x; k < NB; k += T) s_grid[k] = 0.0;
  __syncthreads();
  BoxD b;
  box_derive(S.sc->box, b);
  box_uniform(b);
  const double delvolinv = (double)NG / b.vol;
  const int MD_G *pkey = pppm_keys_of(S);
  const int natoms = S.natoms, rows = (natoms + 63) >> 6, lane = threadIdx.x & 63, step = 2 * (T >> 6);
  const int cy = byc + 4, cz = bzc + 4;
  auto touches = [&](int key) { return key >= 0 && pppm_rel(PP_KEY_Y(key), y0, 2, ny) < cy && pppm_rel(PP_KEY_Z(key), z0, 2, nz) < cz; };
  int r = 2 * ((int)threadIdx.x >> 6);
  for (;;) {
    int aA = 0, kA = 0, kB = 0;
    bool vB = false, found = false;
    for (; r < rows; r += step) {
      const int a = lane * rows + r;
      if (a >= natoms) { r = rows; break; }
      const bool hasB = r + 1 < rows && a + 1 < natoms;
      const int k0 = pkey[a], k1 = hasB ? pkey[a + 1] : -1;
      const bool c0 = touches(k0), c1 = touches(k1);
      if (!c0 && !c1) continue;
      aA = c0 ? a : a + 1; kA = c0 ? k0 : k1;
      vB = c0 && c1; kB = k1;
      found = true;
      r += step;
      break;
    }
    if (!found) break;
    const int aB = aA + 1;
    double wxA[PP_ORDER], wyA[PP_ORDER], wzA[PP_ORDER], wxB[PP_ORDER] = {0, 0, 0, 0, 0}, wyB[PP_ORDER] = {0, 0, 0, 0, 0}, wzB[PP_ORDER] = {0, 0, 0, 0, 0};
    int gxA[PP_ORDER], gyA[PP_ORDER], gzA[PP_ORDER], gxB[PP_ORDER] = {0, 0, 0, 0, 0}, gyB[PP_ORDER] = {0, 0, 0, 0, 0}, gzB[PP_ORDER] = {0, 0, 0, 0, 0};
    double l0, l1, l2;
    atom_lamda(S, b, aA, l0, l1, l2);
    const int ixA = pppm_weights(l0 * nx, wxA);
    pppm_weights_at(l1 * ny, ny, PP_KEY_Y(kA), wyA); pppm_weights_at(l2 * nz, nz, PP_KEY_Z(kA), wzA);
    pppm_wrap(ixA, nx, gxA); pppm_wrap(PP_KEY_Y(kA), ny, gyA); pppm_wrap(PP_KEY_Z(kA), nz, gzA);
    const double zA = delvolinv * S.q[aA];
    double zB = 0.0;
    int ixB = -1000;
    if (vB) {
      atom_lamda(S, b, aB, l0, l1, l2);
      ixB = pppm_weights(l0 * nx, wxB);
      pppm_weights_at(l1 * ny, ny, PP_KEY_Y(kB), wyB); pppm_weights_at(l2 * nz, nz, PP_KEY_Z(kB), wzB);
      pppm_wrap(ixB, nx, gxB); pppm_wrap(PP_KEY_Y(kB), ny, gyB); pppm_wrap(PP_KEY_Z(kB), nz, gzB);
      zB = delvolinv * S.q[aB];
// ... 50 lines not shown
  if (!pppm_brick(nx, ny, nz, budget, 1, B)) return;
  const int y0 = B.y0, z0 = B.z0, byc = B.byc, bzc = B.bzc, hy = B.hy, hz = B.hz;
  const int sy = byc + hy, sz = bzc + hz, SN = nx * sy * sz, T = TPB_;
  const size_t gs = (size_t)S.pgstride;
  const double2 *ex = (const double2 *)S.pfield, *ey = ex + gs, *ez = ey + gs;
  const double *fr = (const double *)S.pfield;
  for (int k = threadIdx.x; k < SN; k += T) {
    const int row = k / nx, x = k - row * nx, j = row / sy, i = row - j * sy;
    const int g = ((hz ? pmod(z0 - 2 + j, nz) : j) * ny + (hy ? pmod(y0 - 2 + i, ny) : i)) * nx + x;
    if (REALF) { s_grid[k] = fr[g]; s_grid[SN + k] = fr[gs + g]; s_grid[2 * SN + k] = fr[2 * gs + g]; }
    else { s_grid[k] = ex[g].x; s_grid[SN + k] = ey[g].x; s_grid[2 * SN + k] = ez[g].x; }
  }
  __syncthreads();
  BoxD b;
  box_derive(S.sc->box, b);
  box_uniform(b);
  const int MD_G *pkey = pppm_keys_of(S);
  const int natoms = S.natoms;
  int a = threadIdx.x;
  for (;;) {
    int key = 0;
    for (; a < natoms; a += T) {
      key = pkey[a];
      if ((unsigned)(PP_KEY_Y(key) - y0) < (unsigned)byc && (unsigned)(PP_KEY_Z(key) - z0) < (unsigned)bzc) break;
    }
    if (a >= natoms) break;
    const int at = a;
    a += T;
    if (key < 0) {
      if (!add) { S.f[3 * at] = 0.0; S.f[3 * at + 1] = 0.0; S.f[3 * at + 2] = 0.0; }
      continue;
    }
    double l0, l1, l2;
    atom_lamda(S, b, at, l0, l1, l2);
    double wx[PP_ORDER], wy[PP_ORDER], wz[PP_ORDER];
    int gx[PP_ORDER], jy[PP_ORDER], jz[PP_ORDER];
    const int iy = PP_KEY_Y(key), iz = PP_KEY_Z(key);
    pppm_wrap(pppm_weights(l0 * nx, wx), nx, gx);
    pppm_weights_at(l1 * ny, ny, iy, wy); pppm_weights_at(l2 * nz, nz, iz, wz);
    pppm_wrap(iy, ny, jy); pppm_wrap(iz, nz, jz);
#pragma unroll
    for (int k = 0; k < PP_ORDER; k++) { if (hy) jy[k] = iy - y0 + k; if (hz) jz[k] = iz - z0 + k; }
    double fx = 0.0, fy = 0.0, fz = 0.0;
#pragma unroll
    for (int c = 0; c < PP_ORDER; c++) {
#pragma unroll
      for (int bb = 0; bb < PP_ORDER; bb++) {
        const double zy = wz[c] * wy[bb];
        const int row = (jz[c] * sy + jy[bb]) * nx;
        double rx = 0.0, ry = 0.0, rz = 0.0;
#pragma unroll
        for (int k = 0; k < PP_ORDER; k++) {
          const int g = row + gx[k];
          rx = fma(wx[k], s_grid[g], rx); ry = fma(wx[k], s_grid[SN + g], ry); rz = fma(wx[k], s_grid[2 * SN + g], rz);
        }
        fx = fma(zy, rx, fx); fy = fma(zy, ry, fy); fz = fma(zy, rz, fz);
      }
    }
    const double qf = MD_QQRD2E * S.q[at];
    if (add) { S.f[3 * at] += qf * fx; S.f[3 * at + 1] += qf * fy; S.f[3 * at + 2] += qf * fz; }
    else { S.f[3 * at] = qf * fx; S.f[3 * at + 1] = qf * fy; S.f[3 * at + 2] = qf * fz; }
  }
}


size_t mdk_pppm_lds_limit() { return 144 * 1024; }
static inline int pppm_split(int ns, int maxatoms) {
  return std::max(1, std::min(std::min(ns < 32 ? 64 : 16, cdiv(2048, ns)), maxatoms / 256));
}
static inline size_t pppm_budget(const PppmLaunch *tl) { return tl && tl->budget > 0 ? (size_t)tl->budget : mdk_pppm_lds_limit(); }
static inline bool pppm_padx(int maxgridp, const PppmLaunch *tl) {
  static const bool padx_off = scema_env("SCEMA_MD_PPPM_PADX") && atoi(scema_env("SCEMA_MD_PPPM_PADX")) == 0;
  return maxgridp > 0 && !padx_off && (size_t)maxgridp * sizeof(double) <= std::min((size_t)36 * 1024, pppm_budget(tl));
}
int mdk_pppm_spread_path(int maxgrid, int maxgridp, const PppmLaunch *tl) {
  const size_t lds = (size_t)(pppm_padx(maxgridp, tl) ? maxgridp : maxgrid) * sizeof(double);
  if (lds <= pppm_budget(tl)) return 0;
  return tl && tl->mode != 0 && tl->sp_tiles > 0 ? 1 : 2;
}
int mdk_pppm_force_path(int maxgrid, const PppmLaunch *tl) {
  if (3 * (size_t)maxgrid * sizeof(double) <= pppm_budget(tl)) return 0;
  return tl && tl->mode != 0 && tl->fo_tiles > 0 ? 1 : 2;
}
void mdk_pppm_keys(hipStream_t st, const SimDev *d, int ns, int maxatoms) { hipLaunchKernelGGL(k_pppm_keys, grid2(cdiv(maxatoms, 256), ns), dim3(256), 0, st, d); }
int mdk_pppm_spread(hipStream_t st, const SimDev *d, int ns, int maxgrid, int maxatoms, int zeroed, int maxgridp, const PppmLaunch *tl) {
  const bool padx = pppm_padx(maxgridp, tl);
  const size_t lds = (size_t)(padx ? maxgridp : maxgrid) * sizeof(double);
  const int path = mdk_pppm_spread_path(maxgrid, maxgridp, tl);
  if (path == 1) {
    const size_t tlds = tl->sp_lds;
    static size_t optin_tab[16] = {0};
    size_t &optin = lds_optin_slot(optin_tab);
    if (tlds > 64 * 1024 && tlds > optin) { (void)hipFuncSetAttribute((const void *)k_pppm_spread_tiled<PP_TPB>, hipFuncAttributeMaxDynamicSharedMemorySize, (int)tlds); optin = tlds; }
    if (tlds <= 36 * 1024) hipLaunchKernelGGL((k_pppm_spread_tiled<256>), grid2(tl->sp_tiles, ns), dim3(256), tlds, st, d, tl->budget);
    else hipLaunchKernelGGL((k_pppm_spread_tiled<PP_TPB>), grid2(tl->sp_tiles, ns), dim3(PP_TPB), tlds, st, d, tl->budget);
    return path;
  }
  const bool use_lds = path == 0;
  const int split = pppm_split(ns, maxatoms);
  if ((!use_lds || split > 1) && !zeroed) hipLaunchKernelGGL(k_pppm_zero, grid2(cdiv(maxgrid, 256), ns), dim3(256), 0, st, d);
  if (!use_lds) {
    hipLaunchKernelGGL((k_pppm_spread<false, 256>), grid2(split, ns), dim3(256), 0, st, d, split);
    return path;
  }
  static size_t optin_tab[16] = {0};
  size_t &optin = lds_optin_slot(optin_tab);
  if (lds > 64 * 1024 && lds > optin) { (void)hipFuncSetAttribute((const void *)k_pppm_spread<true, PP_TPB>, hipFuncAttributeMaxDynamicSharedMemorySize, (int)lds); optin = lds; }
  if (padx) hipLaunchKernelGGL((k_pppm_spread<true, 256, true>), grid2(split, ns), dim3(256), lds, st, d, split);
  else if (lds <= 36 * 1024) hipLaunchKernelGGL((k_pppm_spread<true, 256>), grid2(split, ns), dim3(256), lds, st, d, split);
  else hipLaunchKernelGGL((k_pppm_spread<true, PP_TPB>), grid2(split, ns), dim3(PP_TPB), lds, st, d, split);
  return path;
}
int mdk_pppm_solve_max() { return PP_SOLVE_MAX; }
void mdk_pppm_solve(hipStream_t st, const SimDev *d, int ns, int maxgrid, int maxdims) {
  static const int shape_env = scema_env("SCEMA_MD_PPPM_SOLVE_WIDE") ? atoi(scema_env("SCEMA_MD_PPPM_SOLVE_WIDE")) : -1;
  const bool wide = shape_env < 0 ? ns < 8 : shape_env != 0;
  static const int two_env = scema_env("SCEMA_MD_PPPM_SOLVE_TWO") ? atoi(scema_env("SCEMA_MD_PPPM_SOLVE_TWO")) : -1;
  const bool two = wide && (two_env < 0 ? ns < 8 : two_env != 0);
  const size_t lds = ((wide ? 3 : 2) * (size_t)maxgrid + (size_t)maxdims) * sizeof(double2);
  static size_t optin_tab[2][16] = {{0}, {0}};
  size_t &optin = lds_optin_slot(optin_tab[wide ? 1 : 0]);
  if (wide) {
    if (lds > 64 * 1024 && lds > optin) { (void)hipFuncSetAttribute((const void *)k_pppm_solve<1024, false>, hipFuncAttributeMaxDynamicSharedMemorySize, (int)lds); optin = lds; }
    hipLaunchKernelGGL((k_pppm_solve<1024, false>), dim3(ns, two ? 2 : 1), dim3(1024), lds, st, d);
  } else {
    if (lds > 64 * 1024 && lds > optin) { (void)hipFuncSetAttribute((const void *)k_pppm_solve<512, true>, hipFuncAttributeMaxDynamicSharedMemorySize, (int)lds); optin = lds; }
    hipLaunchKernelGGL((k_pppm_solve<512, true>), dim3(ns), dim3(512), lds, st, d);
  }
}
void mdk_pppm_gf(hipStream_t st, const SimDev *d, int ns, int maxgrid) { hipLaunchKernelGGL(k_pppm_gf, grid2(cdiv(maxgrid, 256), ns), dim3(256), 0, st, d); }
void mdk_pppm_poisson(hipStream_t st, const SimDev *d, int ns, int maxgrid) { hipLaunchKernelGGL(k_pppm_poisson, grid2(cdiv(maxgrid, 256), ns), dim3(256), 0, st, d); }
int mdk_pppm_force(hipStream_t st, const SimDev *d, int ns, int maxgrid, int maxatoms, int add, int real_fields, const PppmLaunch *tl) {
  const size_t lds = 3 * (size_t)maxgrid * sizeof(double);
  const int path = mdk_pppm_force_path(maxgrid, tl);
  if (path == 1) {
    const size_t tlds = tl->fo_lds;
    static size_t optin_tab[16] = {0};
    size_t &optin = lds_optin_slot(optin_tab);
    if (tlds > 64 * 1024 && tlds > optin) {
      (void)hipFuncSetAttribute((const void *)k_pppm_force_tiled<PP_TPB, false>, hipFuncAttributeMaxDynamicSharedMemorySize, (int)tlds);
      (void)hipFuncSetAttribute((const void *)k_pppm_force_tiled<PP_TPB, true>, hipFuncAttributeMaxDynamicSharedMemorySize, (int)tlds);
      optin = tlds;
    }
    const dim3 g = grid2(tl->fo_tiles, ns);
    if (tlds <= 36 * 1024) {
      if (real_fields) hipLaunchKernelGGL((k_pppm_force_tiled<256, true>), g, dim3(256), tlds, st, d, tl->budget, add);
      else hipLaunchKernelGGL((k_pppm_force_tiled<256, false>), g, dim3(256), tlds, st, d, tl->budget, add);
    } else {
      if (real_fields) hipLaunchKernelGGL((k_pppm_force_tiled<PP_TPB, true>), g, dim3(PP_TPB), tlds, st, d, tl->budget, add);
      else hipLaunchKernelGGL((k_pppm_force_tiled<PP_TPB, false>), g, dim3(PP_TPB), tlds, st, d, tl->budget, add);
    }
    return path;
  }
  if (path == 2) {
    if (real_fields) hipLaunchKernelGGL((k_pppm_force<false, true>), grid2(cdiv(maxatoms, 256), ns), dim3(256), 0, st, d, cdiv(maxatoms, 256), add);
    else hipLaunchKernelGGL((k_pppm_force<false, false>), grid2(cdiv(maxatoms, 256), ns), dim3(256), 0, st, d, cdiv(maxatoms, 256), add);
    return path;
  }
  static size_t optin_tab[16] = {0};
  size_t &optin = lds_optin_slot(optin_tab);
  if (lds > 64 * 1024 && lds > optin) {
    (void)hipFuncSetAttribute((const void *)k_pppm_force<true, false>, hipFuncAttributeMaxDynamicSharedMemorySize, (int)lds);
    (void)hipFuncSetAttribute((const void *)k_pppm_force<true, true>, hipFuncAttributeMaxDynamicSharedMemorySize, (int)lds);
    optin = lds;
  }
  const int split = pppm_split(ns, maxatoms);
  if (real_fields) hipLaunchKernelGGL((k_pppm_force<true, true>), grid2(split, ns), dim3(256), lds, st, d, split, add);
  else hipLaunchKernelGGL((k_pppm_force<true, false>), grid2(split, ns), dim3(256), lds, st, d, split, add);
  return path;
}
```

Measured before the change: 471.0 evals/s.

## Bin atoms by nearest grid point for PPPM charge spreading in LDS

Adds a binned charge-assignment path. A new k_pppm_bins kernel groups charged atoms by nearest grid point, using LDS counting sort and a block scan, into work items of up to M atoms. k_pppm_spread_binned then accumulates each group's stencil contributions in registers before issuing one LDS atomic per grid point, which cuts the number of LDS atomics when atoms per grid point is high. The path is chosen by a policy on replica count and charged atoms per grid point, and the scratch buffer is enlarged to hold items and the permutation. The cost is an extra kernel launch with a single-workgroup-per-replica sort pass.

```diff
diff --git a/include/scema_md.h b/include/scema_md.h
--- a/include/scema_md.h
+++ b/include/scema_md.h
@@ -196,6 +196,8 @@
 int scema_md_batch_split(scema_md_engine *e, int32_t on);
 int scema_md_get_concurrency(const scema_md_engine *e, int32_t *out);
 int scema_md_pppm_tiling(scema_md_engine *e, int32_t mode, int32_t lds_bytes);
+int scema_md_pppm_binning(scema_md_engine *e, int32_t mode);
+long long scema_md_pppm_binned_launches(const scema_md_engine *e);
 int scema_md_pppm_paths(const scema_md_engine *e, int32_t out[8]);
 int scema_md_pppm_tile_shape(const int32_t grid[3], int32_t lds_bytes, int32_t which , int32_t out[4]);
 int scema_md_pppm_plan_count(const scema_md_engine *e);
diff --git a/scema_amd/capi.py b/scema_amd/capi.py
--- a/scema_amd/capi.py
+++ b/scema_amd/capi.py
@@ -26,7 +26,7 @@
     "scema_md_comm_world", "scema_md_comm_rank", "scema_md_comm_stats", "scema_md_comm_handshakes", "scema_md_state_owner", "scema_md_last_plan",
     "scema_plan_dir_create", "scema_plan_dir_destroy", "scema_plan_update", "scema_md_kspace_setup",
     "scema_md_save_state_dump", "scema_md_replica_natoms", "scema_md_save_replica_file", "scema_md_equilibrate", "scema_md_debug_minimize", "scema_md_debug_run_nh",
-    "scema_md_reax_configure", "scema_md_reax_activate", "scema_md_reax_set", "scema_md_reax_concurrency", "scema_md_batch_split", "scema_md_get_concurrency", "scema_md_pppm_plan_count", "scema_md_pppm_tiling", "scema_md_pppm_paths", "scema_md_pppm_tile_shape", "scema_md_unsettled_updates", "scema_md_reax_debug_compute", "scema_md_reax_stats", "scema_md_box_fma_tflops",
+    "scema_md_reax_configure", "scema_md_reax_activate", "scema_md_reax_set", "scema_md_reax_concurrency", "scema_md_batch_split", "scema_md_get_concurrency", "scema_md_pppm_plan_count", "scema_md_pppm_tiling", "scema_md_pppm_binning", "scema_md_pppm_binned_launches", "scema_md_pppm_paths", "scema_md_pppm_tile_shape", "scema_md_unsettled_updates", "scema_md_reax_debug_compute", "scema_md_reax_stats", "scema_md_box_fma_tflops",
     "scema_md_sw_configure", "scema_md_sw_debug_compute", "scema_md_sw_read_params",
     "scema_md_tersoff_configure", "scema_md_tersoff_debug_compute", "scema_md_tersoff_read_params",
     "scema_md_eam_configure", "scema_md_eam_debug_compute", "scema_md_eam_read_setfl",
@@ -447,6 +447,13 @@
     def pppm_tiling(self, mode: int = -1, lds_bytes: int = -1):
         self._chk(lib().scema_md_pppm_tiling(self.h, C.c_int32(mode), C.c_int32(lds_bytes)))
 
+    def pppm_binning(self, mode: int = -1):
+        self._chk(lib().scema_md_pppm_binning(self.h, C.c_int32(mode)))
+
+    def pppm_binned_launches(self) -> int:
+        lib().scema_md_pppm_binned_launches.restype = C.c_longlong
+        return int(lib().scema_md_pppm_binned_launches(self.h))
+
     def pppm_paths(self) -> dict:
         out = (C.c_int32 * 8)()
         self._chk(lib().scema_md_pppm_paths(self.h, out))
diff --git a/scema_amd/csrc/engine/engine.h b/scema_amd/csrc/engine/engine.h
--- a/scema_amd/csrc/engine/engine.h
+++ b/scema_amd/csrc/engine/engine.h
@@ -121,6 +121,7 @@
   std::vector<double> q, mass_atom, lj;
   int nbonds = 0, nbonds_noshake = 0, nangles = 0, ndihedrals = 0, nimpropers = 0, nspecial = 0, nclus = 0, ncons = 0, nfree = 0;
   double qsqsum = 0, qsum = 0, excl_cut = 0;
+  int ncharged = 0;
   double init_box[9];
   std::vector<double> init_x, init_v;
   DevBuf d_rtype;
@@ -315,6 +316,8 @@
   std::vector<std::unique_ptr<DevBuf>> bak_x, bak_v;
   int pppm_tile_mode = 1, pppm_lds_bytes = 0;
   int pppm_paths[8] = {0, 0, 0, 0, 0, 0, 0, 1};
+  int pppm_bin_mode = 2;
+  long long pppm_binned_launches = 0;
   std::map<std::array<int, 6>, hipfftHandle> pppm_plans;
   std::vector<int> h_kpack;
   int local_stress_count = 0;
diff --git a/scema_amd/csrc/engine/engine_core.cpp b/scema_amd/csrc/engine/engine_core.cpp
--- a/scema_amd/csrc/engine/engine_core.cpp
+++ b/scema_amd/csrc/engine/engine_core.cpp
@@ -52,6 +52,7 @@
     {"SCEMA_MD_PPPM_SOLVE_WIDE", "1 / 0: the in-LDS PPPM solve with 1 024 threads and three LDS grids / 512 threads and two (default: by batch size)"},
     {"SCEMA_MD_PPPM_SOLVE_TWO", "0 / 1: the in-LDS PPPM solve of the 1 024-thread shape as one / two workgroups per replica, one per transform back (default: two for batches under 8 replicas)"},
     {"SCEMA_MD_PPPM_PADX", "0: the LDS grid of the PPPM spreading kernel without the five pad points per x row (an address addition per stencil point instead of a constant offset)"},
+    {"SCEMA_MD_PPPM_BINNED", "0 / 1: the charge assignment of meshes kept whole in LDS never / wherever eligible as k_pppm_bins + k_pppm_spread_binned, atoms grouped by nearest grid point (default: by launch size and atoms per grid point)"},
     {"SCEMA_MD_PPPM_FFT", "hipFFT for every PPPM grid (default: grids of up to 2 900 points are solved in LDS)"},
     {"SCEMA_MD_FUSED_TAIL", "0 / 1: force assembly + SHAKE + second kick as three kernels / as k_finish (default: by batch size)"},
     {"SCEMA_MD_BONDED_SIDE", "0: the bonded kernel of a small batch always on the main stream behind the pair kernel (default: behind the PPPM chain on the side stream on steps without a new influence function)"},
diff --git a/scema_amd/csrc/engine/engine_reax.cpp b/scema_amd/csrc/engine/engine_reax.cpp
--- a/scema_amd/csrc/engine/engine_reax.cpp
+++ b/scema_amd/csrc/engine/engine_reax.cpp
@@ -395,6 +395,13 @@
   if (lds_bytes >= 0) e->pppm_lds_bytes = lds_bytes;
   return SCEMA_MD_OK;
 }
+int scema_md_pppm_binning(scema_md_engine *e, int32_t mode) {
+  if (!e) return SCEMA_MD_ERR_ARG;
+  if (mode < -1 || mode > 2) return fail(e, SCEMA_MD_ERR_ARG, "scema_md_pppm_binning: mode %d (0 off, 1 wherever eligible, 2 by the launch policy, -1 keeps)", mode);
+  if (mode >= 0) e->pppm_bin_mode = mode;
+  return SCEMA_MD_OK;
+}
+long long scema_md_pppm_binned_launches(const scema_md_engine *e) { return e ? e->pppm_binned_launches : -(long long)SCEMA_MD_ERR_ARG; }
 int scema_md_pppm_paths(const scema_md_engine *e, int32_t out[8]) {
   if (!e || !out) return SCEMA_MD_ERR_ARG;
   for (int k = 0; k < 8; k++) out[k] = e->pppm_paths[k];
diff --git a/scema_amd/csrc/engine/engine_run.cpp b/scema_amd/csrc/engine/engine_run.cpp
--- a/scema_amd/csrc/engine/engine_run.cpp
+++ b/scema_amd/csrc/engine/engine_run.cpp
@@ -92,6 +92,7 @@
   int maxbt = 1, maxloc = 1, maxcoef = 0, maxrow = 64, maxcapj = 64, maxpoly = 1, maxatoms = 0, maxpad = 0, maxcells = 0, maxk = 0, mmax = 1,
       maxgrp = 0, maxclus = 0, maxunits = 0, maxsteps = 0;
   int maxgrid = 0, maxgridp = 0, maxdims = 0;
+  long long sum_charged = 0, sum_grid = 0;
   bool padx_ok = true;
   PppmLaunch tl;
   bool tl_sp_fits = true, tl_fo_fits = true;
@@ -321,6 +322,7 @@
     for (int d = 0; d < 3; d++) S.pg[d] = -ew.kmaxd[d];
     L.maxgrid = std::max(L.maxgrid, S.pg[0] * S.pg[1] * S.pg[2]);
     if (S.pg[0] < 5) L.padx_ok = false;
+    L.sum_charged += T.ncharged; L.sum_grid += (long long)S.pg[0] * S.pg[1] * S.pg[2];
     L.maxgridp = std::max(L.maxgridp, (S.pg[0] + 5) * S.pg[1] * S.pg[2]);
     for (int which = 0; which < 2; which++) {
       const PppmTile t = pppm_tile_shape(S.pg[0], S.pg[1], S.pg[2], L.tl.budget, which);
@@ -438,7 +440,7 @@
   if (!L.tl_fo_fits) L.tl.fo_tiles = 0;
   if (L.maxgrid > 0) {
     const size_t mg = (size_t)L.maxgrid;
-    const size_t gfs = mg + ((size_t)L.maxatoms + 1) / 2;
+    const size_t gfs = mg + (3 * (size_t)L.maxatoms + 2 + 1) / 2;
     HIPCHK(e->d_pppm.ensure((size_t)ns * (mg * 4 * sizeof(double2) + gfs * sizeof(double))));
     double *gbase = e->d_pppm.as<double>(), *ebase = gbase + (size_t)ns * mg * 2, *fbase = gbase + (size_t)ns * mg * 8;
     for (int pos = 0; pos < ns; pos++) {
@@ -485,7 +487,15 @@
     std::memcpy(e->pppm_paths, paths, sizeof paths);
   }
   if (sp_path == 1 || fo_path == 1) mdk_pppm_keys(st, Dp, na, L.maxatoms);
-  mdk_pppm_spread(st, Dp, na, L.maxgrid, L.maxatoms, clean ? 1 : 0, maxgridp, &L.tl);
+  static const int binned_env = scema_env("SCEMA_MD_PPPM_BINNED") ? (atoi(scema_env("SCEMA_MD_PPPM_BINNED")) != 0 ? 1 : 0) : -1;
+  const int bin_mode = binned_env >= 0 ? binned_env : e->pppm_bin_mode;
+  PppmLaunch tl = L.tl;
+  if (bin_mode != 0 && mdk_pppm_binned_ok(L.maxgrid, maxgridp, &L.tl)) {
+    const PppmBinPolicy bp;
+    tl.binned = bin_mode == 1 || (na >= bp.min_replicas && (double)L.sum_charged >= bp.min_per_point * (double)L.sum_grid) ? 1 : 0;
+  }
+  if (tl.binned) e->pppm_binned_launches += 1;
+  mdk_pppm_spread(st, Dp, na, L.maxgrid, L.maxatoms, clean ? 1 : 0, maxgridp, &tl);
   clean = false;
   if (pol.pppm_in_lds) {
     if (new_box) mdk_pppm_gf(st, Dp, na, L.maxgrid);
diff --git a/scema_amd/csrc/engine/engine_topo.cpp b/scema_amd/csrc/engine/engine_topo.cpp
--- a/scema_amd/csrc/engine/engine_topo.cpp
+++ b/scema_amd/csrc/engine/engine_topo.cpp
@@ -31,6 +31,7 @@
     t.type[i] = cls[s->type[i]];
     t.mass_atom[i] = s->mass[s->type[i]];
     t.qsqsum += t.q[i] * t.q[i];
+    t.ncharged += t.q[i] != 0.0 ? 1 : 0;
     t.qsum += t.q[i];
   }
   const int nt2 = ncls * ncls;
diff --git a/scema_amd/csrc/md_pppm.h b/scema_amd/csrc/md_pppm.h
--- a/scema_amd/csrc/md_pppm.h
+++ b/scema_amd/csrc/md_pppm.h
@@ -6,7 +6,10 @@
   int budget = 0, mode = 1;
   int sp_ty = 0, sp_tz = 0, sp_tiles = 0, fo_ty = 0, fo_tz = 0, fo_tiles = 0;
   size_t sp_lds = 0, fo_lds = 0;
+  int binned = 0;
 };
+struct PppmBinPolicy { int min_replicas = 72; double min_per_point = 2.0; };
+int mdk_pppm_binned_ok(int maxgrid, int maxgridp, const PppmLaunch *tl);
 int mdk_pppm_spread_path(int maxgrid, int maxgridp, const PppmLaunch *tl);
 int mdk_pppm_force_path(int maxgrid, const PppmLaunch *tl);
 void mdk_pppm_keys(hipStream_t st, const SimDev *d, int ns, int maxatoms);
diff --git a/scema_amd/csrc/md_pppm.hip b/scema_amd/csrc/md_pppm.hip
--- a/scema_amd/csrc/md_pppm.hip
+++ b/scema_amd/csrc/md_pppm.hip
@@ -48,10 +48,13 @@
 #pragma unroll
     for (int k = 0; k < PP_ORDER; k++) g[k] = pmod(i + k - 2, n);
 }
-__device__ __forceinline__ void atom_lamda(const SimDev &S, const BoxD &b, int a, double &t0, double &t1, double &t2) {
-  const double d0 = S.x[3 * a] - b.lo[0], d1 = S.x[3 * a + 1] - b.lo[1], d2 = S.x[3 * a + 2] - b.lo[2];
+__device__ __forceinline__ void pos_lamda(const BoxD &b, double x0, double x1, double x2, double &t0, double &t1, double &t2) {
+  const double d0 = x0 - b.lo[0], d1 = x1 - b.lo[1], d2 = x2 - b.lo[2];
   const double l0 = b.hinv[0] * d0 + b.hinv[5] * d1 + b.hinv[4] * d2, l1 = b.hinv[1] * d1 + b.hinv[3] * d2, l2 = b.hinv[2] * d2;
   t0 = l0 - floor(l0); t1 = l1 - floor(l1); t2 = l2 - floor(l2);
+}
+__device__ __forceinline__ void atom_lamda(const SimDev &S, const BoxD &b, int a, double &t0, double &t1, double &t2) {
+  pos_lamda(b, S.x[3 * a], S.x[3 * a + 1], S.x[3 * a + 2], t0, t1, t2);
 }
 
 __global__ __launch_bounds__(256) void k_pppm_zero(const SimDev *sims) {
@@ -61,6 +64,35 @@
 }
 
 extern __shared__ double s_grid[];
+template <bool PADX>
+__device__ __forceinline__ void pppm_grid_out(const SimDev &S, int nx, int ny, int nz, int split) {
+  const int NG = nx * ny * nz, T = (int)blockDim.x, nxp = PADX ? nx + 5 : nx;
+  double2 *rho = (double2 *)S.pgrid;
+  __syncthreads();
+  if (PADX) {
+    const int nrow = ny * nz;
+    for (int k = threadIdx.x; k < 5 * nrow; k += T) {
+      const int row = k / 5, pc = k - 5 * row;
+      const int src = pc < 2 ? pc : nx + pc, dst = (pc < 2 ? nx - 2 + pc : pc - 2) + 2;
+      s_grid[row * nxp + dst] += s_grid[row * nxp + src];
+    }
+    __syncthreads();
+    for (int k = threadIdx.x; k < NG; k += T) {
+      const int row = k / nx, x = k - row * nx;
+      const double v = s_grid[row * nxp + x + 2];
+      if (split == 1) rho[k] = make_double2(v, 0.0);
+      else if (v != 0.0) atomicAdd(&rho[k].x, v);
+    }
+  } else if (split == 1) {
+    for (int k = threadIdx.x; k < NG; k += T) rho[k] = make_double2(s_grid[k], 0.0);
+  } else {
+    for (int k = threadIdx.x; k < NG; k += T) {
+      const double v = s_grid[k];
+      if (v != 0.0) atomicAdd(&rho[k].x, v);
+    }
+  }
+}
+
 template <bool LDS, int TPB_, bool PADX = false>
 __global__ __launch_bounds__(TPB_) void k_pppm_spread(const SimDev *sims, int split) {
   const SimDev &S = sims[blockIdx.y];
@@ -138,31 +170,189 @@
       }
     }
   }
-  if (LDS) {
-    __syncthreads();
-    if (PADX) {
-      const int nrow = ny * nz;
-      for (int k = threadIdx.x; k < 5 * nrow; k += T) {
-        const int row = k / 5, pc = k - 5 * row;
-        const int src = pc < 2 ? pc : nx + pc, dst = (pc < 2 ? nx - 2 + pc : pc - 2) + 2;
-        s_grid[row * nxp + dst] += s_grid[row * nxp + src];
-      }
-      __syncthreads();
-      for (int k = threadIdx.x; k < NG; k += T) {
-        const int row = k / nx, x = k - row * nx;
-        const double v = s_grid[row * nxp + x + 2];
-        if (split == 1) rho[k] = make_double2(v, 0.0);
-        else if (v != 0.0) atomicAdd(&rho[k].x, v);
-      }
-    } else if (split == 1) {
-      for (int k = threadIdx.x; k < NG; k += T) rho[k] = make_double2(s_grid[k], 0.0);
-    } else {
-      for (int k = threadIdx.x; k < NG; k += T) {
-        const double v = s_grid[k];
-        if (v != 0.0) atomicAdd(&rho[k].x, v);
-      }
-    }
-  }
+  if (LDS) pppm_grid_out<PADX>(S, nx, ny, nz, split);
+}
+
+__device__ __forceinline__ int MD_G *pppm_keys_of(const SimDev &S) { return (int MD_G *)(S.pgf + S.pgstride); }
+
+#ifndef PP_BIN_M
+#define PP_BIN_M 4
+#endif
+#define PP_BIN_TPB 1024
+#define PP_BIN_ROUNDS 4
+#define PP_BIN_BATCH 4
+extern __shared__ int s_bins[];
+template <int NV>
+__device__ __forceinline__ void pppm_block_scan(int (&v)[NV], int (&tot)[NV], int *lds ) {
+  constexpr int NW = PP_BIN_TPB / 64;
+  const int lane = threadIdx.x & 63, wave = threadIdx.x >> 6;
+  int inc[NV];
+#pragma unroll
+  for (int i = 0; i < NV; i++) {
+    int x = v[i];
+#pragma unroll
+    for (int d = 1; d < 64; d <<= 1) {
+      const int y = __shfl_up(x, d);
+      if (lane >= d) x += y;
+    }
+    inc[i] = x;
+    if (lane == 63) lds[i * NW + wave] = x;
+  }
+  __syncthreads();
+#pragma unroll
+  for (int i = 0; i < NV; i++) {
+    int before = 0, all = 0;
+    for (int w = 0; w < NW; w++) { const int t = lds[i * NW + w]; all += t; if (w < wave) before += t; }
+    v[i] = before + inc[i] - v[i];
+    tot[i] = all;
+  }
+  __syncthreads();
+}
+__global__ __launch_bounds__(PP_BIN_TPB) void k_pppm_bins(const SimDev *sims, int M) {
+  const SimDev &S = sims[blockIdx.x];
+  const int nx = S.pg[0], ny = S.pg[1], nz = S.pg[2];
+  if (nx == 0) return;
+  const int nbx = nx + 1, nbins = nbx * ny * nz, natoms = S.natoms;
+  int *s_cnt = s_bins, *s_start = s_bins + nbins;
+  __shared__ int s_scan[(PP_BIN_ROUNDS + 1) * (PP_BIN_TPB / 64)];
+  int MD_G *head = pppm_keys_of(S);
+  int2 MD_G *items = (int2 MD_G *)(head + 2);
+  int MD_G *perm = head + 2 + 2 * (size_t)natoms;
+  for (int k = threadIdx.x; k < nbins; k += PP_BIN_TPB) s_cnt[k] = 0;
+  __syncthreads();
+  BoxD b;
+  box_derive(S.sc->box, b);
+  box_uniform(b);
+  for (int a0 = threadIdx.x; a0 < natoms; a0 += PP_BIN_BATCH * PP_BIN_TPB) {
+    double q[PP_BIN_BATCH], x0[PP_BIN_BATCH], x1[PP_BIN_BATCH], x2[PP_BIN_BATCH];
+#pragma unroll
+    for (int j = 0; j < PP_BIN_BATCH; j++) {
+      const int a = min(a0 + j * PP_BIN_TPB, natoms - 1);
+      q[j] = S.q[a]; x0[j] = S.x[3 * a]; x1[j] = S.x[3 * a + 1]; x2[j] = S.x[3 * a + 2];
+    }
+#pragma unroll
+    for (int j = 0; j < PP_BIN_BATCH; j++) {
+      const int a = a0 + j * PP_BIN_TPB;
+      if (a >= natoms) break;
+      int bin = -1, rank = 0;
+      if (q[j] != 0.0) {
+        double l0, l1, l2;
+        pos_lamda(b, x0[j], x1[j], x2[j], l0, l1, l2);
+        const int ix = min(max(pppm_nearest(l0 * nx), 0), nx), iy = pmod(pppm_nearest(l1 * ny), ny), iz = pmod(pppm_nearest(l2 * nz), nz);
+        bin = (iz * ny + iy) * nbx + ix;
+        rank = atomicAdd(&s_cnt[bin], 1);
+      }
+      items[a] = make_int2(bin, rank);
+    }
+  }
+  __syncthreads();
+  const int per = (nbins + PP_BIN_TPB - 1) / PP_BIN_TPB, b0 = min(nbins, (int)threadIdx.x * per), b1 = min(nbins, b0 + per);
+  int v[PP_BIN_ROUNDS + 1], tot[PP_BIN_ROUNDS + 1];
+#pragma unroll
+  for (int r = 0; r <= PP_BIN_ROUNDS; r++) v[r] = 0;
+  for (int k = b0; k < b1; k++) {
+    const int n = s_cnt[k], parts = (n + M - 1) / M;
+    v[PP_BIN_ROUNDS] += n;
+#pragma unroll
+    for (int r = 0; r < PP_BIN_ROUNDS - 1; r++) v[r] += parts > r ? 1 : 0;
+    v[PP_BIN_ROUNDS - 1] += max(parts - (PP_BIN_ROUNDS - 1), 0);
+  }
+  pppm_block_scan<PP_BIN_ROUNDS + 1>(v, tot, s_scan);
+  {
+    int at = v[PP_BIN_ROUNDS];
+    for (int k = b0; k < b1; k++) { s_start[k] = at; at += s_cnt[k]; }
+  }
+  __syncthreads();
+  for (int a0 = threadIdx.x; a0 < natoms; a0 += PP_BIN_BATCH * PP_BIN_TPB) {
+    int2 br[PP_BIN_BATCH];
+#pragma unroll
+    for (int j = 0; j < PP_BIN_BATCH; j++) br[j] = items[min(a0 + j * PP_BIN_TPB, natoms - 1)];
+#pragma unroll
+    for (int j = 0; j < PP_BIN_BATCH; j++) {
+      const int a = a0 + j * PP_BIN_TPB;
+      if (a < natoms && br[j].x >= 0) perm[s_start[br[j].x] + br[j].y] = a;
+    }
+  }
+  __syncthreads();
+  {
+    int at[PP_BIN_ROUNDS], base = 0;
+#pragma unroll
+    for (int r = 0; r < PP_BIN_ROUNDS; r++) { at[r] = base + v[r]; base += tot[r]; }
+    if (threadIdx.x == 0) head[0] = base;
+    for (int k = b0; k < b1; k++) {
+      const int n = s_cnt[k], first = s_start[k];
+      for (int p = 0, left = n; left > 0; p++, left -= M) {
+        int idx = 0;
+#pragma unroll
+        for (int r = 0; r < PP_BIN_ROUNDS; r++)
+          if (min(p, PP_BIN_ROUNDS - 1) == r) idx = at[r]++;
+        items[idx] = make_int2(k | (min(left, M) << 24), first + p * M);
+      }
+    }
+  }
+}
+
+template <int M>
+__global__ __launch_bounds__(256) void k_pppm_spread_binned(const SimDev *sims, int split) {
+  const SimDev &S = sims[blockIdx.y];
+  const int nx = S.pg[0], ny = S.pg[1], nz = S.pg[2];
+  if (nx == 0) return;
+  const int NG = nx * ny * nz, nxp = nx + 5, NGP = nxp * ny * nz, nbx = nx + 1;
+  const int MD_G *head = pppm_keys_of(S);
+  const int2 MD_G *items = (const int2 MD_G *)(head + 2);
+  const int MD_G *perm = head + 2 + 2 * (size_t)S.natoms;
+  const int nitems = head[0];
+  const int chunk = (nitems + split - 1) / split, i0 = (int)blockIdx.x * chunk, i1 = min(nitems, i0 + chunk);
+  if (i0 >= i1 && split > 1) return;
+  BoxD b;
+  box_derive(S.sc->box, b);
+  box_uniform(b);
+  for (int k = threadIdx.x; k < NGP; k += 256) s_grid[k] = 0.0;
+  __syncthreads();
+  const double delvolinv = (double)NG / b.vol;
+  for (int it = i0 + (int)threadIdx.x; it < i1; it += 256) {
+    const int2 item = items[it];
+    const int bin = item.x & 0xffffff, n = item.x >> 24, first = item.y;
+    const int rowb = bin / nbx, ix = bin - rowb * nbx, iz = rowb / ny, iy = rowb - iz * ny;
+    int at[M];
+    double px[M], py[M], pz[M], zq[M];
+#pragma unroll
+    for (int j = 0; j < M; j++) at[j] = perm[first + min(j, n - 1)];
+#pragma unroll
+    for (int j = 0; j < M; j++) {
+      px[j] = S.x[3 * at[j]]; py[j] = S.x[3 * at[j] + 1]; pz[j] = S.x[3 * at[j] + 2];
+      zq[j] = j < n ? delvolinv * S.q[at[j]] : 0.0;
+    }
+    double wx[M][PP_ORDER], wy[M][PP_ORDER], wz[M][PP_ORDER];
+#pragma unroll
+    for (int j = 0; j < M; j++) {
+      double l0, l1, l2;
+      pos_lamda(b, px[j], py[j], pz[j], l0, l1, l2);
+      pppm_blend(0.5 - ((double)ix - l0 * nx), wx[j]);
+      pppm_weights_at(l1 * ny, ny, iy, wy[j]); pppm_weights_at(l2 * nz, nz, iz, wz[j]);
+#pragma unroll
+      for (int k = 0; k < PP_ORDER; k++) wx[j][k] *= zq[j];
+    }
+    int gy[PP_ORDER], gz[PP_ORDER];
+    pppm_wrap(iy, ny, gy); pppm_wrap(iz, nz, gz);
+#pragma unroll
+    for (int c = 0; c < PP_ORDER; c++) {
+#pragma unroll
+      for (int bb = 0; bb < PP_ORDER; bb++) {
+        double acc[PP_ORDER] = {0, 0, 0, 0, 0};
+#pragma unroll
+        for (int j = 0; j < M; j++) {
+          const double zy = wz[j][c] * wy[j][bb];
+#pragma unroll
+          for (int k = 0; k < PP_ORDER; k++) acc[k] = fma(zy, wx[j][k], acc[k]);
+        }
+        double *prow = s_grid + (gz[c] * ny + gy[bb]) * nxp + ix;
+#pragma unroll
+        for (int k = 0; k < PP_ORDER; k++) (void)__hip_atomic_fetch_add(prow + k, acc[k], __ATOMIC_RELAXED, __HIP_MEMORY_SCOPE_WORKGROUP);
+      }
+    }
+  }
+  pppm_grid_out<true>(S, nx, ny, nz, split);
 }
 
 __device__ __forceinline__ double sinc_pow10(double x) {
@@ -443,7 +633,6 @@
 
 #define PP_KEY_Y(key) ((key) & 0xffff)
 #define PP_KEY_Z(key) (((key) >> 16) & 0x7fff)
-__device__ __forceinline__ int MD_G *pppm_keys_of(const SimDev &S) { return (int MD_G *)(S.pgf + S.pgstride); }
 __global__ __launch_bounds__(256) void k_pppm_keys(const SimDev *sims) {
   const SimDev &S = sims[blockIdx.y];
   if (S.pg[0] == 0) return;
@@ -660,6 +849,9 @@
   if (3 * (size_t)maxgrid * sizeof(double) <= pppm_budget(tl)) return 0;
   return tl && tl->mode != 0 && tl->fo_tiles > 0 ? 1 : 2;
 }
+int mdk_pppm_binned_ok(int maxgrid, int maxgridp, const PppmLaunch *tl) {
+  return mdk_pppm_spread_path(maxgrid, maxgridp, tl) == 0 && pppm_padx(maxgridp, tl) && mdk_pppm_force_path(maxgrid, tl) != 1;
+}
 void mdk_pppm_keys(hipStream_t st, const SimDev *d, int ns, int maxatoms) { hipLaunchKernelGGL(k_pppm_keys, grid2(cdiv(maxatoms, 256), ns), dim3(256), 0, st, d); }
 int mdk_pppm_spread(hipStream_t st, const SimDev *d, int ns, int maxgrid, int maxatoms, int zeroed, int maxgridp, const PppmLaunch *tl) {
   const bool padx = pppm_padx(maxgridp, tl);
@@ -677,6 +869,11 @@
   const bool use_lds = path == 0;
   const int split = pppm_split(ns, maxatoms);
   if ((!use_lds || split > 1) && !zeroed) hipLaunchKernelGGL(k_pppm_zero, grid2(cdiv(maxgrid, 256), ns), dim3(256), 0, st, d);
+  if (tl && tl->binned && mdk_pppm_binned_ok(maxgrid, maxgridp, tl)) {
+    hipLaunchKernelGGL(k_pppm_bins, dim3(ns), dim3(PP_BIN_TPB), 2 * (size_t)maxgridp * sizeof(int), st, d, PP_BIN_M);
+    hipLaunchKernelGGL((k_pppm_spread_binned<PP_BIN_M>), grid2(split, ns), dim3(256), lds, st, d, split);
+    return path;
+  }
   if (!use_lds) {
     hipLaunchKernelGGL((k_pppm_spread<false, 256>), grid2(split, ns), dim3(256), 0, st, d, split);
     return path;
```

After: 477.9 evals/s, median of 6. 1.5% higher.
